# surftemp/cae_tools

Measured on AMD Instinct MI355X. Metric: train images/sec (16x16->256x256, batch 64), higher is better.
Workload: dtype f32

## Files before the change

### cae_tools_amd/csrc/engine.hip

```cpp
#include <hip/hip_runtime.h>

#include <dlfcn.h>

#include <algorithm>
#include <cmath>
#include <cstdio>
#include <cstdlib>
#include <cstring>
#include <map>
#include <string>
#include <tuple>
#include <vector>

#include "cae_hip.h"
#include "kernels_generic.h"
#include "kernels_s2.h"
#include "kernels_last.h"
#include "kernels_rows.h"
#include "kernels_gemm.h"
#include "kernels_igemm.h"
#include "kernels_ctlds.h"
#include "kernels_head.h"
#include "dp_comm.h"
#include "kernels_ctbwd.h"
#include "trunk_api.h"
#include "engine_host.h"

namespace cae {
template __global__ void k_ct_fwd_lds<3, 3>(CtFwd);
template __global__ void k_s2_fwd_rows<8, 4, 1, 2>(S2FwdRows);
template __global__ void k_s2_fwd_rows<4, 2, 2, 1>(S2FwdRows);
template __global__ void k_s2_last_fused<2, 1, 4, 4, 4, true, true>(S2Last);
template __global__ void k_s2_bwd_rows<4, 4, 2, 3, 3, 2, 1, 3>(S2Rows);
template __global__ void k_s2_bwd_rows<8, 2, 4, 3, 3, 4, 2, 1>(S2Rows);
}

using namespace cae;
using namespace cae_internal;

namespace cae_internal {
int ctbwd_launch(const void* args, size_t bytes, unsigned gx, unsigned gy, unsigned gz, size_t lds, hipStream_t s);
}

namespace {
thread_local std::string g_err;
}

void cae_detail_set_error(const char* msg) { g_err = msg; }

namespace {

constexpr float kBnEps = 1e-5f;
constexpr float kBnMomentum = 0.1f;
constexpr int kLossSlots = 1 << 16;

int64_t align_up(int64_t v, int64_t a) { return (v + a - 1) / a * a; }

struct ConvLayer {
    bool transposed;
    int cin, hin, win, cout, hout, wout, kh, kw, stride, opad;
    bool has_bn;
    int bn_index;
    int64_t w_off, b_off, gamma_off, beta_off;
    int64_t rm_off, rv_off;
    int64_t act_off, grad_off;
    int sh_w = -1, sh_b = -1;
    int64_t out_elems() const { return (int64_t)cout * hout * wout; }
    int64_t in_elems() const { return (int64_t)cin * hin * win; }
};

struct FcLayer {
    int nin, nout;
    int64_t w_off, b_off;
    int64_t act_off, grad_off;
    bool relu;
};

}

struct cae_engine {
    std::vector<ConvLayer> enc, dec;
    FcLayer fc[4];
    int fc_size = 0, latent = 0, max_batch = 0;
    int in_c = 0, in_h = 0, in_w = 0, out_c = 0, out_h = 0, out_w = 0;
    TensorTable tab;
    int n_bn = 0;
    std::vector<int64_t> bn_stat_off;
    std::vector<int64_t> bn_saved_off;
    std::vector<int> bn_channels;
    int max_channels = 0;

    int64_t off_state = 0, off_losses = 0, off_zero_begin = 0, off_gradacc = 0, off_zero_end = 0;
    int64_t off_glast = 0, off_sgacc = 0;
    ShardSegs segs{};
    int64_t ws_need = 0;

    float *params = nullptr, *grads = nullptr, *m = nullptr, *v = nullptr, *bufs = nullptr;
    char* ws = nullptr;
    hipStream_t stream = nullptr;
    Hyper hp{1e-3, 0.9, 0.999, 1e-8, 1e-5};
    const float* ds_x[2] = {nullptr, nullptr};
    const float* ds_t[2] = {nullptr, nullptr};
    int64_t ds_n[2] = {0, 0};
    bool graph_mode = true;
    bool lr_stale = true;
    long long captures = 0;
    bool capture_only = false;
    bool use_s2 = true;
    bool variational = false;
    int64_t off_vz = 0, off_vgz = 0, off_zlast = 0;
    cae_internal::TrunkHooks hooks{nullptr, nullptr, nullptr};
    bool gather_fwd = false;
    int ctbwd_mask = 0;
    int ctbwd_auto = 0;
    int64_t off_xbatch = 0;
    bool x_published = false;
    AdamConv0 c0_pending{};
    bool profiling = false;
    struct ProfRec { const char* name; int layer; double bytes; hipEvent_t e0, e1; };
    std::vector<ProfRec> prof;
    std::map<std::tuple<int, int, int, int, const void*, int, int, int, int, int>, hipGraphExec_t> graphs;

    int dp_world = 0, dp_rank = 0;
    RcclApi::comm_t dp_comm = nullptr;
    hipStream_t comm_stream = nullptr;
    hipEvent_t ev_fork = nullptr, ev_join = nullptr;
    bool dp_graph_ok = true;
    bool dp_overlap = true;
    std::vector<int> sync_order;
    size_t sync_pos = 0;
    int64_t bucket_split = 0;

    StepState* state() const { return reinterpret_cast<StepState*>(ws + off_state); }
    double* losses() const { return reinterpret_cast<double*>(ws + off_losses); }
    double* gradacc() const { return reinterpret_cast<double*>(ws + off_gradacc); }
    double* sgacc() const { return reinterpret_cast<double*>(ws + off_sgacc); }
    ShardSegs shard_segs() const {
        ShardSegs r = segs;
        r.base = sgacc();
        return r;
    }
    double* bn_stats(int j) const { return reinterpret_cast<double*>(ws + bn_stat_off[j]); }
    float* bn_saved(int j) const { return reinterpret_cast<float*>(ws + bn_saved_off[j]); }
    float* fptr(int64_t off) const { return reinterpret_cast<float*>(ws + off); }
    void drop_graphs() {
        for (auto& kv : graphs) (void)hipGraphExecDestroy(kv.second);
        graphs.clear();
    }
};

namespace {


BnDesc bn_none() {
    BnDesc d;
    memset(&d, 0, sizeof d);
    d.mode = BN_NONE;
    return d;
}

BnDesc bn_of(const cae_engine* e, const ConvLayer& L, int mode, double count, int update) {
    if (!L.has_bn) return bn_none();
    BnDesc d;
    memset(&d, 0, sizeof d);
    d.mode = mode;
    d.C = L.cout;
    d.stats = e->bn_stats(L.bn_index);
    d.gamma = e->params + L.gamma_off;
    d.beta = e->params + L.beta_off;
    d.rmean = e->bufs + L.rm_off;
    d.rvar = e->bufs + L.rv_off;
    d.saved = e->bn_saved(L.bn_index);
    d.count = count;
    d.inv_count = count > 0.0 ? 1.0 / count : 0.0;
    d.unbias = count > 1.0 ? count / (count - 1.0) : 1.0;
    d.momentum = kBnMomentum;
    d.eps = kBnEps;
    d.update = update;
    return d;
}

Src src_plain(const float* p, int C, int H, int W) {
    Src s;
    memset(&s, 0, sizeof s);
    s.p = p;
    s.C = C;
    s.H = H;
    s.W = W;
    return s;
}

Epi epi_plain(float* out) {
    Epi e;
    memset(&e, 0, sizeof e);
// ... 342 lines not shown
}

constexpr int kLastHB = 4;

struct LastPick { bool vec4, bn; };

int last_strips(const ConvLayer& L) {
    const int qw = (L.wout + 1) / 2;
    const int wmax = L.win > qw - 1 ? L.win : qw - 1;
    return (wmax + kLastStripPx - 1) / kLastStripPx;
}

LastPick choose_last(const ConvLayer& L, bool bn_in) { return LastPick{last_strips(L) == 1 && (L.wout & 3) == 0, bn_in}; }

template <int CIN, int COUT, int KH, int KW>
bool last_fused_launch(S2Last a, LastPick p, hipStream_t s) {
    if constexpr (CIN * COUT * KH * KW <= 72) {
        a.QH = (a.OH + 1) / 2;
        a.QW = (a.OW + 1) / 2;
        const int wmax = a.W > a.QW - 1 ? a.W : a.QW - 1, hmax = a.H > a.QH - 1 ? a.H : a.QH - 1;
        a.strips = (wmax + kLastStripPx - 1) / kLastStripPx;
        a.bands = (hmax + kLastHB - 1) / kLastHB;
        a.total = a.B * a.strips * a.bands;
        const dim3 grid((a.total + 3) / 4);
        if (p.vec4 && p.bn) hipLaunchKernelGGL((k_s2_last_fused<CIN, COUT, KH, KW, kLastHB, true, true>), grid, dim3(256), 0, s, a);
        else if (p.bn) hipLaunchKernelGGL((k_s2_last_fused<CIN, COUT, KH, KW, kLastHB, false, true>), grid, dim3(256), 0, s, a);
        else hipLaunchKernelGGL((k_s2_last_fused<CIN, COUT, KH, KW, kLastHB, false, false>), grid, dim3(256), 0, s, a);
        return true;
    }
    return false;
}

bool last_fused_dispatch(const ConvLayer& L, const S2Last& a, hipStream_t s) {
    const LastPick p = choose_last(L, a.bn_in.mode != BN_NONE);
#define ONE(CI, CO, KH_, KW_) \
    if (L.cin == CI && L.cout == CO && L.kh == KH_ && L.kw == KW_) return last_fused_launch<CI, CO, KH_, KW_>(a, p, s);
#define PAIR(CI, CO) S2_KERNELS(ONE, CI, CO)
    S2_SHAPES(PAIR)
#undef PAIR
#undef ONE
    return false;
}

template <class K>
void head_lds_attr(K kernel, size_t bytes) {
    static size_t granted = 64 * 1024;
    if (bytes > granted) {
        (void)hipFuncSetAttribute(reinterpret_cast<const void*>(kernel), hipFuncAttributeMaxDynamicSharedMemorySize, (int)bytes);
        granted = bytes;
    }
}

template <int KH, int KW>
void ct_fwd_go(const CtFwd& c, dim3 grid, int threads, size_t lds, hipStream_t s) {
    head_lds_attr(k_ct_fwd_lds<KH, KW>, lds);
    hipLaunchKernelGGL((k_ct_fwd_lds<KH, KW>), grid, dim3(threads), lds, s, c);
}

constexpr int kCtFwdMfmas = 24;

bool ct_fwd_plan(const cae_engine* e, int batch, const ConvLayer& L, int layer, CtFwd& c, int& waves, size_t& lds) {
    if (e->gather_fwd || layer >= 31 || L.cin % 4 || L.kh < 3 || L.kw < 3) return false;
    memset(&c, 0, sizeof c);
    c.B = batch; c.Cin = L.cin; c.H = L.hin; c.W = L.win; c.Cout = L.cout; c.OH = L.hout; c.OW = L.wout;
    c.QH = (L.hout + 1) / 2; c.QW = (L.wout + 1) / 2;
    c.PW = c.QW + 1;
    c.plane = ((c.QH + 1) * c.PW) | 1;
    c.tiles = (c.QH * c.QW + 15) / 16;
    const int taps = ((L.kh + 1) / 2 + L.kh / 2) * ((L.kw + 1) / 2 + L.kw / 2);
    const int mf = L.cin * taps / 4;
    int ks = 1;
    while (ks < 8 && mf / ks > kCtFwdMfmas && L.cin % (ks * 2 * 4) == 0) ks *= 2;
    int rt = 8 / ks;
    if (rt > c.tiles) rt = c.tiles;
    if (rt > 4) rt = 4;
    c.ks = ks; c.rt = rt;
    c.tg = (c.tiles + rt - 1) / rt;
    waves = rt * ks;
    lds = ct_fwd_lds_bytes(L.cin, c.plane, L.kh, L.kw, waves, ks);
    return !(lds > 150 * 1024 || c.plane >= kDivSmallMaxD || (long long)L.cin * c.plane >= kDivSmallMaxN);
}

void ct_fwd_launch(cae_engine* e, const StepArgs& a, const ConvLayer& L, int layer, const float* in, const BnDesc& bn_in,
                   float* out, double* stats) {
    CtFwd c;
    int waves = 0;
    size_t lds = 0;
    (void)ct_fwd_plan(e, a.batch, L, layer, c, waves, lds);
    c.in = in; c.bn_in = bn_in; c.w = e->params + L.w_off; c.bias = e->params + L.b_off; c.out = out; c.stats = stats;
    dim3 grid((unsigned)(a.batch * c.tg), (unsigned)((L.cout + 15) / 16));
    ProfScope _p(e, a.train ? "ct_convt_fwd" : "ct_convt_eval", layer, f4((double)a.batch * (L.in_elems() + L.out_elems())));
    if (L.kh == 3 && L.kw == 3) ct_fwd_go<3, 3>(c, grid, 64 * waves, lds, e->stream);
    else if (L.kh == 4 && L.kw == 4) ct_fwd_go<4, 4>(c, grid, 64 * waves, lds, e->stream);
    else if (L.kh == 3 && L.kw == 4) ct_fwd_go<3, 4>(c, grid, 64 * waves, lds, e->stream);
    else ct_fwd_go<4, 3>(c, grid, 64 * waves, lds, e->stream);
}

struct CtBwdPlan { int imgs, groups, wstr; size_t lds; };

bool ct_bwd_plan(const cae_engine* e, int B, const ConvLayer& L, int l, CtBwdPlan& p) {
    if (!(l < 31 && ((e->ctbwd_mask >> l) & 1) && L.kh == 3 && L.kw == 3 && L.stride == 2 && L.cin % 16 == 0 && L.cout % 4 == 0 &&
          L.hout >= 2 * L.hin + 1 && L.wout >= 2 * L.win + 1))
        return false;
    const int HW = L.hin * L.win, OHW = L.hout * L.wout, N = L.cout * 9;
    const int budget = std::min((4 * kCtbG4 * kCtbThreads) / (L.cout * OHW), (4 * kCtbA4 * kCtbThreads) / (16 * HW));
    int imgs = (int)(((int64_t)L.cin * N * B + 149999) / 150000);
    imgs = std::max(1, std::min(std::min(imgs, budget), B));
    p.imgs = imgs;
    p.groups = (B + imgs - 1) / imgs;
    p.wstr = N | 1;
    p.lds = ct_bwd_lds_bytes(L.cin, L.cout, imgs, HW, OHW, p.wstr);
    return budget >= 1 && 16 * N <= 4 * kCtbW4 * kCtbThreads && p.lds <= 152 * 1024 && (int64_t)L.cin * N * p.groups <= 400000;
}


bool head_plan(const cae_engine* e, const StepArgs& a, HeadArgs& h, size_t& lds_bytes) {
    if (!e->use_s2 || a.syncing() || e->variational || (int)e->enc.size() > kHeadMaxEnc) return false;
    memset(&h, 0, sizeof h);
    h.B = a.batch;
    h.n_enc = (int)e->enc.size();
    h.train = a.train ? 1 : 0;
    h.momentum = kBnMomentum;
    h.eps = kBnEps;
    h.st = e->state();
    h.tiles_per_wg = 1;
    double* acc = e->gradacc();
    int64_t top = 0;
    auto take = [&](int64_t floats) {
        top = align_up(top, 4);
        const int64_t o = top;
        top += floats;
        return (int)o;
    };
    h.o_perm = take(a.batch);
    int maxc = 1;
    for (int l = 0; l < h.n_enc; l++) {
        const ConvLayer& L = e->enc[l];
        if (L.cout > kHeadMaxC) return false;
        HeadConv& c = h.enc[l];
        c.cin = L.cin; c.hin = L.hin; c.win = L.win; c.cout = L.cout; c.hout = L.hout; c.wout = L.wout;
        c.kh = L.kh; c.kw = L.kw; c.s = L.stride;
        c.w = e->params + L.w_off; c.bias = e->params + L.b_off;
        c.gamma = e->params + L.gamma_off; c.beta = e->params + L.beta_off;
        c.rmean = e->bufs + L.rm_off; c.rvar = e->bufs + L.rv_off; c.saved = e->bn_saved(L.bn_index);
        c.y = e->fptr(L.act_off);
        {
            const double count = (double)a.batch * L.hout * L.wout;
            c.inv_count = 1.0 / count;
            c.unbias = count > 1.0 ? count / (count - 1.0) : 1.0;
        }
        {
            const int64_t pn = L.beta_off + L.cout - L.w_off, bnn = L.rv_off + L.cout - L.rm_off;
            if (pn > kHeadThreads || bnn > kHeadThreads || pn <= 0 || bnn <= 0 || h.n_seg + 2 > kHeadMaxSeg) return false;
            c.o_w = take(pn);
            c.o_b = c.o_w + (int)(L.b_off - L.w_off);
            c.o_gamma = c.o_w + (int)(L.gamma_off - L.w_off);
            c.o_beta = c.o_w + (int)(L.beta_off - L.w_off);
            c.o_rm = take(bnn);
            c.o_rv = c.o_rm + (int)(L.rv_off - L.rm_off);
            h.seg[h.n_seg++] = HeadSeg{e->params + L.w_off, (int)pn, c.o_w, 0};
            h.seg[h.n_seg++] = HeadSeg{e->bufs + L.rm_off, (int)bnn, c.o_rm, 0};
        }
        c.o_c = take(4 * (int64_t)L.cout);
        if (l + 1 == h.n_enc) c.o_y = take((int64_t)a.batch * L.out_elems());
        if (L.cout > maxc) maxc = L.cout;
    }
    int maxd = 0;
    for (int i = 0; i < 4; i++) {
        const FcLayer& F = e->fc[i];
        HeadFc& f = h.fc[i];
        f.nin = F.nin; f.nout = F.nout; f.relu = F.relu ? 1 : 0;
        f.w = e->params + F.w_off; f.bias = e->params + F.b_off;
// ... 96 lines not shown
    t.ld2 = ld_of(e->fc[2].nout);
    t.ld1 = ld_of(e->fc[1].nout);
    t.ld0 = ld_of(e->fc[0].nout);
    int64_t top = 0;
    auto take = [&](int64_t floats) {
        top = align_up(top, 4);
        const int64_t o = top;
        top += floats;
        return (int)o;
    };
    t.o_c = take(4 * (int64_t)P.cout);
    t.o_red = take(2 * 2 * (int64_t)kHeadWaves);
    t.o_g2 = take(16 * (int64_t)t.ld2 + 32);
    t.o_g1 = take(16 * (int64_t)t.ld1 + 32);
    t.o_g0 = take(16 * (int64_t)t.ld0 + 32);
    t.o_y = take(16 * (int64_t)e->fc[0].nin + 32);
    t.o_gx = take(16 * (int64_t)e->fc[0].nin + 32);
    top = align_up(top, 4);
    t.zero4 = (int)((top - t.o_g2) / 4);
    int64_t wmax = 0;
    for (int i = 0; i < 3; i++) wmax = std::max<int64_t>(wmax, (int64_t)e->fc[i].nout * t.ldw[i]);
    t.o_w = take(wmax + 64);
    t.o_part = take(kHeadWaves * 256);
    lds_bytes = (size_t)align_up(top, 4) * sizeof(float);
    if (lds_bytes > 152 * 1024) return false;
    for (int i = 0; i < 3; i++) t.sp_d[i] = stage_split((e->fc[2 - i].nin + 15) / 16, e->fc[2 - i].nout);
    for (int i = 0; i < 3; i++) t.sp_w[i] = stage_split(((e->fc[2 - i].nout + 15) / 16) * ((e->fc[2 - i].nin + 16) / 16), 16);
    return true;
}

enum DecFwdK {
    DF_FUSED_LAST,
    DF_ROWS,
    DF_S2,
    DF_CT_LDS,
    DF_IG,
    DF_UP
};
enum DecBwdK {
    DB_FUSED_LAST,
    DB_ROWS,
    DB_S2,
    DB_CT_LDS,
    DB_IG,
    DB_GENERIC
};

int s2_fwd_epi(const cae_engine* e, int l, bool train, bool external_loss) {
    if (l + 1 < (int)e->dec.size()) return train ? S2_RAW_STATS : S2_RAW;
    if (external_loss) return S2_RAW;
    return train ? S2_SIGMSE : S2_SIGOUT;
}

bool rows_ok(const cae_engine* e, const ConvLayer& L, int l) {
    return l + 1 < (int)e->dec.size() && l > 0 && e->dec[l - 1].has_bn && rows_bwd_ok(e, L);
}

DecFwdK choose_dec_fwd(const cae_engine* e, const ConvLayer& L, int l, int B, bool train, bool external_loss) {
    const bool last = l + 1 == (int)e->dec.size();
    if (last && train && !external_loss && last_fused_ok(e, L)) return DF_FUSED_LAST;
    if (rows_ok(e, L, l)) return DF_ROWS;
    if (s2_eligible(e, L)) return DF_S2;
    if (e->use_s2 && !last && L.stride == 2 && L.kh <= 4 && L.kw <= 4) {
        CtFwd c;
        int waves = 0;
        size_t lds = 0;
        return ct_fwd_plan(e, B, L, l, c, waves, lds) ? DF_CT_LDS : DF_IG;
    }
    return DF_UP;
}

DecBwdK choose_dec_bwd(const cae_engine* e, const ConvLayer& L, int l, int B, bool external_loss) {
    const bool last = l + 1 == (int)e->dec.size();
    if (last && !external_loss && last_fused_ok(e, L)) return DB_FUSED_LAST;
    if (rows_ok(e, L, l)) return DB_ROWS;
    if (s2_eligible(e, L)) return DB_S2;
    if (e->use_s2) {
        CtBwdPlan p;
        return ct_bwd_plan(e, B, L, l, p) ? DB_CT_LDS : DB_IG;
    }
    return DB_GENERIC;
}

StepTail narrow_tail(cae_engine* e, bool with_step_tail, int batch_inc) {
    StepTail t = step_tail_of(e, batch_inc, 1);
    if (!with_step_tail) {
        t.zero_extra = nullptr;
        t.zero_extra_n = 0;
        t.st = nullptr;
    }
    return t;
}

int dp_allreduce_grads(cae_engine* e, int64_t lo, int64_t hi, hipStream_t on) {
    if (hi <= lo) return CAE_OK;
    NCCL_TRY(rccl().AllReduce(e->grads + lo, e->grads + lo, (size_t)(hi - lo), RcclApi::kFloat32, RcclApi::kSum, e->dp_comm, on));
    return CAE_OK;
}

bool dp_overlap(const cae_engine* e, const StepArgs& a) { return e->dp_overlap && !a.dp_sync; }

bool dp_single_collective(const cae_engine* e, const StepArgs& a) { return !dp_overlap(e, a) && !a.dp_sync; }

int dp_first_bucket(cae_engine* e, const StepArgs& a) {
    if (!a.dp || dp_single_collective(e, a)) return CAE_OK;
    const int64_t lo = e->bucket_split, hi = e->tab.n_param;
    const bool overlap = dp_overlap(e, a);
    hipStream_t on = overlap ? e->comm_stream : e->stream;
    if (overlap) {
        HIP_TRY(hipEventRecord(e->ev_fork, e->stream));
        HIP_TRY(hipStreamWaitEvent(e->comm_stream, e->ev_fork, 0));
    }
    {
        ProfScope _p(e, "dp_narrow_bucket0", 0, 12.0 * (hi - lo), on);
        hipLaunchKernelGGL(k_narrow_range, dim3(grid1(hi - lo)), dim3(256), 0, on, (long long)lo, (long long)hi, e->grads,
                           e->shard_segs(), narrow_tail(e, false, 0));
    }
    if (int rc = dp_allreduce_grads(e, lo, hi, on)) return rc;
    if (overlap) HIP_TRY(hipEventRecord(e->ev_join, e->comm_stream));
    return CAE_OK;
}

int dp_finish_step(cae_engine* e, const StepArgs& a) {
    hipStream_t s = e->stream;
    const int64_t lo = 0, hi = dp_single_collective(e, a) ? e->tab.n_param : e->bucket_split;
    {
        ProfScope _p(e, "dp_narrow_bucket1", 0, 12.0 * (hi - lo));
        hipLaunchKernelGGL(k_narrow_range, dim3(grid1(hi - lo > 0 ? hi - lo : 1)), dim3(256), 0, s, (long long)lo, (long long)hi,
                           e->grads, e->shard_segs(), narrow_tail(e, true, a.inc()));
    }
    if (dp_overlap(e, a)) HIP_TRY(hipStreamWaitEvent(s, e->ev_join, 0));
    if (int rc = dp_allreduce_grads(e, lo, hi, s)) return rc;
    StepTail none;
    memset(&none, 0, sizeof none);
    ProfScope _p(e, "adam", 0, 28.0 * e->tab.n_param);
    hipLaunchKernelGGL(k_adam, dim3(grid1(e->tab.n_param)), dim3(256), 0, s, (long long)e->tab.n_param, e->params,
                       (const float*)e->grads, e->m, e->v, e->hp, (const StepState*)e->state(), e->shard_segs(), none, 0,
                       std::log(e->hp.beta1), std::log(e->hp.beta2), AdamConv0{});
    return CAE_OK;
}

int launch_forward(cae_engine* e, const StepArgs& a) {
    hipStream_t s = e->stream;
    const int B = a.batch;
    const StepState* st = e->state();
    const int act_mode = a.train ? BN_BATCH : BN_RUNNING;

    HeadArgs head;
    size_t head_lds = 0;
    const bool fused_head = a.part == 0 && head_plan(e, a, head, head_lds);
    if (fused_head) {
        head.x = a.x_direct ? a.x_direct : e->ds_x[a.which];
        head.perm = a.x_direct ? nullptr : a.perm;
        head.use_cursor = a.x_direct ? 0 : 1;
        head.bump_adam = a.train ? 1 : 0;
        const int T = (e->fc[3].nout + 15) / 16;
        double bytes = 0;
        for (auto& L : e->enc) bytes += f4((double)B * (L.in_elems() + L.out_elems()));
        for (int i = 0; i < 4; i++) bytes += f4((double)B * (e->fc[i].nin + e->fc[i].nout) + (double)e->fc[i].nin * e->fc[i].nout);
        head_lds_attr(k_head_fwd, head_lds);
        e->x_published = false;
        if (a.train) {
            head.clear0 = e->bn_stats(e->enc[0].bn_index);
            head.clear0_n = kStatShards * e->enc[0].cout * 4;
            if (a.adam_follows) {
                head.xbatch = e->fptr(e->off_xbatch);
// ... 42 lines not shown
        const int fc_lo = a.part == 2 ? 2 : 0, fc_hi = a.part == 1 ? 2 : 4;
        for (int i = fc_lo; i < fc_hi; i++) {
            const FcLayer& F = e->fc[i];
            ProfScope _p(e, e->use_s2 ? "linear_fwd_mfma" : "linear_fwd", i, f4((double)B * (F.nin + F.nout) + (double)F.nin * F.nout));
            if (e->use_s2) {
                GemmArgs ga;
                memset(&ga, 0, sizeof ga);
                ga.M = B; ga.N = F.nout; ga.K = F.nin;
                ga.A = in; ga.sa_m = F.nin; ga.sa_k = 1;
                ga.B = e->params + F.w_off; ga.sb_k = 1; ga.sb_n = F.nin;
                ga.C = e->fptr(F.act_off); ga.sc_m = F.nout; ga.sc_n = 1;
                ga.epi = GE_STORE;
                ga.bias = e->params + F.b_off;
                ga.relu = F.relu ? 1 : 0;
                ga.bn_a = i == 0 ? bni : bn_none();
                ga.hw_a = hw;
                ga.bn_c = bn_none();
                const int tiles = ((B + 15) / 16) * ((F.nout + 15) / 16);
                hipLaunchKernelGGL(k_gemm16, dim3(tiles), dim3(256), gemm_lds(i == 0 ? P.cout : 0), s, ga);
            } else {
                hipLaunchKernelGGL(k_lin_fwd, dim3(grid1((int64_t)B * F.nout)), dim3(256), lds_bytes(i == 0 ? P.cout : 0, 0),
                                   s, B, F.nin, F.nout, in, i == 0 ? bni : bn_none(), hw, e->params + F.w_off,
                                   e->params + F.b_off, F.relu ? 1 : 0, e->fptr(F.act_off));
            }
            in = e->fptr(F.act_off);
            if (i == 1 && e->variational) {
                if (!e->hooks.reparam) return fail(CAE_ERR_STATE, "trunk engine without a reparameterisation hook");
                e->hooks.reparam(e->hooks.user, s, in, B, e->latent, a.train ? 1 : 0, e->fptr(e->off_vz));
                in = e->fptr(e->off_vz);
            }
        }
        if (a.part == 1) {
            HIP_TRY(hipMemcpyAsync(a.z_out, e->fptr(e->fc[1].act_off), sizeof(float) * (size_t)B * e->fc[1].nout, hipMemcpyDeviceToDevice, s));
            return CAE_OK;
        }
    }
    for (size_t l = 0; l < e->dec.size(); l++) {
        const ConvLayer& L = e->dec[l];
        const bool last = l + 1 == e->dec.size();
        ConvGeom g{B, L.cin, L.hin, L.win, L.cout, L.hout, L.wout, L.kh, L.kw, L.stride};
        Src small;
        BnDesc bns = bn_none();
        if (l == 0) {
            small = src_plain(e->fptr(e->fc[3].act_off), L.cin, L.hin, L.win);
        } else {
            const ConvLayer& P = e->dec[l - 1];
            small = src_plain(e->fptr(P.act_off), L.cin, L.hin, L.win);
            bns = bn_of(e, P, act_mode, (double)a.bn_batch * P.hout * P.wout, 1);
        }
        Epi ep;
        if (!last) {
            ep = epi_plain(e->fptr(L.act_off));
            if (a.train) {
                ep.kind = EPI_STATS;
                ep.stats = e->bn_stats(L.bn_index);
                ep.stats_C = L.cout;
            }
        } else {
            memset(&ep, 0, sizeof ep);
            ep.inv_count = (float)(1.0 / ((double)a.global_batch * L.cout * L.hout * L.wout));
            ep.losses = e->losses();
            ep.perm = a.perm;
            ep.use_cursor = a.use_cursor ? 1 : 0;
            if (a.train) {
                ep.kind = EPI_SIGMSE;
                ep.out = e->fptr(e->off_glast);
                ep.target = e->ds_t[a.which];
                ep.bias_acc = e->gradacc() + L.b_off;
            } else {
                ep.kind = EPI_SIGOUT;
                ep.yhat = a.yhat;
                ep.target = a.want_loss ? e->ds_t[a.which] : nullptr;
            }
        }
        if (last && a.external_loss) {
            ep = epi_plain(e->fptr(e->off_zlast));
        }
        const DecFwdK fk = choose_dec_fwd(e, L, (int)l, B, a.train, a.external_loss);
        if (fk == DF_FUSED_LAST) continue;
        if (fk == DF_ROWS) {
            S2FwdRows f;
            memset(&f, 0, sizeof f);
            f.B = B; f.H = L.hin; f.W = L.win; f.OH = L.hout; f.OW = L.wout;
            f.in = small.p; f.bn_in = bns;
            f.w = e->params + L.w_off; f.bias = e->params + L.b_off;
            f.out = ep.out;
            f.stats = a.train ? ep.stats : nullptr;
            ProfScope _p(e, a.train ? "s2_convt_fwd" : "s2_convt_eval", (int)l, f4((double)B * (L.in_elems() + L.out_elems())));
            rows_fwd_launch(L, f, s);
            if (a.train)
                if (int rc = sync_bn_table(e, a, L.bn_index)) return rc;
            continue;
        }
        if (fk == DF_S2) {
            S2Fwd f;
            memset(&f, 0, sizeof f);
            f.B = B; f.H = L.hin; f.W = L.win; f.OH = L.hout; f.OW = L.wout;
            f.in = small.p;
            f.w = e->params + L.w_off;
            f.bias = e->params + L.b_off;
            f.bn_in = bns;
            f.st = st;
            if (!last) {
                f.out = ep.out;
                f.stats = ep.stats;
                f.epi = a.train ? S2_RAW_STATS : S2_RAW;
            } else if (a.external_loss) {
                f.out = ep.out;
                f.epi = S2_RAW;
            } else {
                f.out = a.train ? ep.out : ep.yhat;
                f.target = ep.target;
                f.perm = ep.perm;
                f.use_cursor = ep.use_cursor;
                f.losses = ep.losses;
                f.inv_count = ep.inv_count;
                f.bias_acc = e->sgacc() + L.sh_b;
                f.bias_stride = e->segs.n;
                f.epi = a.train ? S2_SIGMSE : S2_SIGOUT;
            }
            ProfScope _p(e, last ? (a.train ? "s2_convt_last_fwd_loss" : "s2_convt_last_eval") : (a.train ? "s2_convt_fwd" : "s2_convt_eval"), (int)l,
                         f4((double)B * (L.in_elems() + L.out_elems() * (last && (a.train || a.want_loss) ? 2.0 : 1.0))));
            if (!s2_fwd_dispatch(L, f, s))
                return fail(CAE_ERR_STATE, "decoder layer %d: no k_s2_fwd kernel for the chosen variant", (int)l);
            if (a.train && !last)
                if (int rc = sync_bn_table(e, a, L.bn_index)) return rc;
            continue;
        }
        if (fk == DF_CT_LDS) {
            ct_fwd_launch(e, a, L, (int)l, small.p, bns, ep.out, a.train ? ep.stats : nullptr);
            if (a.train)
                if (int rc = sync_bn_table(e, a, L.bn_index)) return rc;
            continue;
        }
        if (fk == DF_IG) {
            IgFwd f;
            memset(&f, 0, sizeof f);
            f.B = B; f.Cin = L.cin; f.H = L.hin; f.W = L.win; f.Cout = L.cout; f.OH = L.hout; f.OW = L.wout;
            f.KH = L.kh; f.KW = L.kw; f.QH = (L.hout + 1) / 2; f.QW = (L.wout + 1) / 2;
            f.in = small.p; f.bn_in = bns; f.w = e->params + L.w_off; f.bias = e->params + L.b_off;
            f.out = ep.out; f.stats = a.train ? ep.stats : nullptr;
            const int mtiles = (B * f.QH * f.QW + 15) / 16;
            f.ksplit = L.cin >= 48 ? 4 : (L.cin >= 24 ? 2 : 1);
            {
                const int waves_m = 4 / f.ksplit, target = 1024;
                int tpw = (mtiles * 4 + waves_m * target - 1) / (waves_m * target);
                f.tiles_per_wave = tpw < 1 ? 1 : (tpw > 8 ? 8 : tpw);
            }
            const int per_block = (4 / f.ksplit) * f.tiles_per_wave;
            dim3 grid((mtiles + per_block - 1) / per_block, 4, (L.cout + 15) / 16);
            ProfScope _p(e, a.train ? "ig_convt_fwd" : "ig_convt_eval", (int)l, f4((double)B * (L.in_elems() + L.out_elems())));
            hipLaunchKernelGGL(k_ig_fwd_s2, grid, dim3(256), (64 + 1024) * sizeof(float) + (size_t)(L.cin + 1) * sizeof(float4), s, f);
            if (a.train)
                if (int rc = sync_bn_table(e, a, L.bn_index)) return rc;
            continue;
        }
        dim3 grid(grid1((int64_t)B * L.hout * L.wout), L.cout);
        ProfScope _p(e, last ? (a.train ? "dec_convt_last_fwd_loss" : "dec_convt_last_eval") : (a.train ? "dec_convt_fwd" : "dec_convt_eval"), (int)l,
                     f4((double)B * (L.in_elems() + L.out_elems() * (last && (a.train || a.want_loss) ? 2.0 : 1.0))));
        hipLaunchKernelGGL(k_up, grid, dim3(256), lds_bytes(L.cin, L.cout), s, g, small, bns, e->params + L.w_off,
                           e->params + L.b_off, ep, bn_none(), st);
        if (a.train && !last)
            if (int rc = sync_bn_table(e, a, L.bn_index)) return rc;
    }
    return CAE_OK;
}

int launch_backward(cae_engine* e, const StepArgs& a) {
    hipStream_t s = e->stream;
    const int B = a.batch;
    const StepState* st = e->state();
    double* acc = e->gradacc();

    for (int l = (int)e->dec.size() - 1; l >= 0; l--) {
        const ConvLayer& L = e->dec[l];
        const bool last = l + 1 == (int)e->dec.size();
        const DecBwdK bk = choose_dec_bwd(e, L, l, B, a.external_loss);
        ConvGeom g{B, L.cin, L.hin, L.win, L.cout, L.hout, L.wout, L.kh, L.kw, L.stride};
        Src gy;
        BnDesc bng = bn_none();
        if (last) {
            gy = src_plain(e->fptr(e->off_glast), L.cout, L.hout, L.wout);
        } else {
            gy = src_plain(e->fptr(L.grad_off), L.cout, L.hout, L.wout);
            gy.q = e->fptr(L.act_off);
            bng = bn_of(e, L, BN_BWD, (double)a.bn_batch * L.hout * L.wout, 0);
        }
        Src ain;
        BnDesc bna = bn_none();
        if (l == 0) {
            ain = src_plain(e->fptr(e->fc[3].act_off), L.cin, L.hin, L.win);
        } else {
            const ConvLayer& P = e->dec[l - 1];
            ain = src_plain(e->fptr(P.act_off), L.cin, L.hin, L.win);
            bna = bn_of(e, P, BN_SAVED, 0, 0);
        }
        if (bk == DB_FUSED_LAST) {
            S2Last f;
            memset(&f, 0, sizeof f);
            f.B = B; f.H = L.hin; f.W = L.win; f.OH = L.hout; f.OW = L.wout;
            f.in = ain.p;
            f.w = e->params + L.w_off;
            f.bias = e->params + L.b_off;
            f.target = e->ds_t[a.which];
            f.perm = a.perm;
            f.use_cursor = a.use_cursor ? 1 : 0;
            f.st = st;
            f.losses = e->losses();
            f.inv_count = (float)(1.0 / ((double)a.global_batch * L.cout * L.hout * L.wout));
            f.bias_acc = e->sgacc() + L.sh_b;
            f.wacc = e->sgacc() + L.sh_w;
            f.acc_stride = e->segs.n;
            if (l == 0) {
                f.bn_in = bn_none();
                f.gin = e->fptr(e->fc[3].grad_off);
            } else {
                const ConvLayer& P = e->dec[l - 1];
                f.bn_in = bn_of(e, P, BN_BATCH, (double)a.bn_batch * P.hout * P.wout, 1);
                f.gin = e->fptr(P.grad_off);
                f.stats_in = e->bn_stats(P.bn_index);
            }
            ProfScope _p(e, "s2_convt_last_fused", l, f4((double)B * (L.in_elems() * 2.0 + L.out_elems())));
            if (!last_fused_dispatch(L, f, s))
                return fail(CAE_ERR_STATE, "decoder layer %d: no k_s2_last_fused kernel for the chosen variant", (int)l);
            if (l > 0)
                if (int rc = sync_bn_table(e, a, e->dec[l - 1].bn_index)) return rc;
            continue;
        }
        if (bk == DB_ROWS) {
            const ConvLayer& P = e->dec[l - 1];
            S2Rows f;
            memset(&f, 0, sizeof f);
            f.B = B; f.H = L.hin; f.W = L.win; f.OH = L.hout; f.OW = L.wout;
            f.g = gy.p; f.yout = gy.q; f.bn_out = bng;
            f.ain = ain.p; f.bn_in = bna;
            f.w = e->params + L.w_off;
            f.gin = e->fptr(P.grad_off);
            f.stats_in = e->bn_stats(P.bn_index);
            f.wacc = e->sgacc() + L.sh_w;
            f.wacc_stride = e->segs.n;
            f.bg.stats = e->bn_stats(L.bn_index);
            f.bg.gamma_acc = acc + L.gamma_off;
            f.bg.beta_acc = acc + L.beta_off;
            f.bg.C = L.cout;
            f.bg.scale = 1.0 / a.world;
            ProfScope _p(e, "s2_convt_bwd", l, f4((double)B * (L.out_elems() * 2.0 + L.in_elems() * 2.0)));
            rows_bwd_launch(L, f, s);
            if (int rc = sync_bn_table(e, a, P.bn_index)) return rc;
            continue;
        }
        if (bk == DB_S2) {
            S2Bwd f;
            memset(&f, 0, sizeof f);
            f.B = B; f.H = L.hin; f.W = L.win; f.OH = L.hout; f.OW = L.wout;
            f.g = gy.p;
            f.yout = gy.q;
            f.bn_out = bng;
            f.ain = ain.p;
            f.bn_in = bna;
            f.w = e->params + L.w_off;
            f.wacc = e->sgacc() + L.sh_w;
            f.wacc_stride = e->segs.n;
            if (l == 0) {
                f.gin = e->fptr(e->fc[3].grad_off);
            } else {
                const ConvLayer& P = e->dec[l - 1];
                f.gin = e->fptr(P.grad_off);
                f.stats_in = e->bn_stats(P.bn_index);
            }
            if (L.has_bn) {
                f.bg.stats = e->bn_stats(L.bn_index);
                f.bg.gamma_acc = acc + L.gamma_off;
                f.bg.beta_acc = acc + L.beta_off;
                f.bg.C = L.cout;
                f.bg.scale = 1.0 / a.world;
            }
            ProfScope _p(e, "s2_convt_bwd", l,
                         f4((double)B * (L.out_elems() * (last ? 1.0 : 2.0) + L.in_elems() * 2.0)));
            if (!s2_bwd_dispatch(L, f, s))
                return fail(CAE_ERR_STATE, "decoder layer %d: no k_s2_bwd kernel for the chosen variant", (int)l);
            if (l > 0)
                if (int rc = sync_bn_table(e, a, e->dec[l - 1].bn_index)) return rc;
            continue;
        }
        if (bk == DB_CT_LDS) {
            CtBwdPlan cp;
            (void)ct_bwd_plan(e, B, L, l, cp);
            const int HW = L.hin * L.win, OHW = L.hout * L.wout;
            const int imgs = cp.imgs, groups = cp.groups, wstr = cp.wstr;
            const size_t lds = cp.lds;
            CtBwd c;
            memset(&c, 0, sizeof c);
            c.B = B; c.Cin = L.cin; c.H = L.hin; c.W = L.win; c.Cout = L.cout; c.OH = L.hout; c.OW = L.wout;
            c.imgs = imgs; c.wstr = wstr;
            c.g = gy.p; c.yout = gy.q; c.bn_out = bng;
            c.ain = ain.p; c.bn_in = bna;
            c.w = e->params + L.w_off;
            if (L.sh_w >= 0) {
                c.wacc = e->sgacc() + L.sh_w;
                c.wacc_stride = e->segs.n;
            } else {
                c.wacc = acc + L.w_off;
            }
            if (l == 0) {
                c.gin = e->fptr(e->fc[3].grad_off);
            } else {
                const ConvLayer& P = e->dec[l - 1];
                c.gin = e->fptr(P.grad_off);
                c.stats_prev = e->bn_stats(P.bn_index);
            }
            if (L.has_bn) {
                c.bg.stats = e->bn_stats(L.bn_index);
                c.bg.gamma_acc = acc + L.gamma_off;
                c.bg.beta_acc = acc + L.beta_off;
                c.bg.C = L.cout;
                c.bg.scale = 1.0 / a.world;
            }
            ProfScope _p(e, "ct_convt_bwd", l,
                         f4((double)B * (L.out_elems() * (last ? 1.0 : 2.0) + L.in_elems() * (l == 0 ? 1.0 : 2.0))));
            int parts = std::max(1, std::min(8, 256 / (groups * (L.cin / 16))));
            size_t lds_launch = lds;
            if (imgs == 1 && parts > 1) {
                const int hb = (L.hin + parts - 1) / parts, bands = (L.hin + hb - 1) / hb;
                const int gstr = (2 * hb + 1) * L.wout, astr = hb * L.win;
                if (bands > 1 && L.cout * gstr <= 8 * kCtbThreads && 16 * astr <= 2 * kCtbThreads) {
                    c.bands = bands;
                    c.hb = hb;
                    parts = bands;
                    lds_launch = (32 * (size_t)kCtbWaves + 4 * (size_t)(L.cin + L.cout) + (size_t)L.cout * gstr + 4 + 16 * (size_t)astr + 4 +
                                  16 * (size_t)wstr + 3 * (size_t)astr + (size_t)kCtbWaves * 16 * 17 + 8) * sizeof(float);
                }
            }
            if (cae_internal::ctbwd_launch(&c, sizeof c, (unsigned)groups, (unsigned)(L.cin / 16), (unsigned)parts, lds_launch, s))
                return fail(CAE_ERR_ARG, "k_ct_bwd_lds: argument layout mismatch");
            if (l > 0)
                if (int rc = sync_bn_table(e, a, e->dec[l - 1].bn_index)) return rc;
            continue;
        }
        if (bk == DB_IG) {
            IgWgrad fw;
            memset(&fw, 0, sizeof fw);
            fw.B = B; fw.Cin = L.cin; fw.H = L.hin; fw.W = L.win; fw.Cout = L.cout; fw.OH = L.hout; fw.OW = L.wout;
            fw.KH = L.kh; fw.KW = L.kw; fw.S = L.stride;
            fw.ain = ain.p; fw.bn_in = bna; fw.g = gy.p; fw.yout = gy.q; fw.bn_out = bng;
            fw.wacc = acc + L.w_off;
            if (L.has_bn) {
                fw.bg.stats = e->bn_stats(L.bn_index);
                fw.bg.gamma_acc = acc + L.gamma_off;
                fw.bg.beta_acc = acc + L.beta_off;
                fw.bg.C = L.cout;
                fw.bg.scale = 1.0 / a.world;
            }
            const int wtiles = ((L.cin + 15) / 16) * ((L.cout * L.kh * L.kw + 15) / 16);
            const int steps = (B * L.hin * L.win + 3) / 4;
            int chunks = 2048 / wtiles;
            if (chunks < 1) chunks = 1;
            int per = (steps + chunks - 1) / chunks;
            per = (per + 31) / 32 * 32;
            chunks = (steps + per - 1) / per;
            fw.ksteps_per_block = per;

            IgDgrad fd;
            memset(&fd, 0, sizeof fd);
            fd.B = B; fd.Cin = L.cin; fd.H = L.hin; fd.W = L.win; fd.Cout = L.cout; fd.OH = L.hout; fd.OW = L.wout;
            fd.KH = L.kh; fd.KW = L.kw; fd.S = L.stride;
            fd.g = gy.p; fd.yout = gy.q; fd.bn_out = bng; fd.w = e->params + L.w_off;
            if (l == 0) {
                fd.gin = e->fptr(e->fc[3].grad_off);
            } else {
                const ConvLayer& P = e->dec[l - 1];
                fd.gin = e->fptr(P.grad_off);
                fd.yprev = e->fptr(P.act_off);
                fd.bn_prev = bn_of(e, P, BN_SAVED, 0, 0);
                fd.stats_prev = e->bn_stats(P.bn_index);
            }
            const int mtiles = (B * L.hin * L.win + 15) / 16;
            const int ksteps = (L.cout * L.kh * L.kw + 3) / 4;
            fd.ksplit = ksteps > 24 ? 4 : (ksteps > 12 ? 2 : 1);
            fd.tiles_per_wave = mtiles >= 8192 ? 2 : 1;
            const int per_block = (4 / fd.ksplit) * fd.tiles_per_wave;
            const int d_gx = (mtiles + per_block - 1) / per_block, d_gy = (L.cin + 15) / 16;
            const size_t lds_d = (128 + 1024) * sizeof(float) + (size_t)(L.cin + L.cout + 1) * sizeof(float4) +
                                 (size_t)L.cout * L.kh * L.kw * 2 * sizeof(int);
            const size_t lds_w = 1024 * sizeof(float) + (size_t)(L.cin + L.cout + 1) * sizeof(float4);
            ProfScope _p(e, "ig_convt_bwd_pair", l,
                         f4((double)B * (L.out_elems() * (last ? 1.0 : 2.0) + L.in_elems() * (l == 0 ? 1.0 : 2.0))));
            int d_group = (per * 4) / (per_block * 16);
            if (d_group < 1) d_group = 1;
            const int w_n8 = (chunks + 7) / 8, d_n8 = ((d_gx + d_group - 1) / d_group + 7) / 8;
            hipLaunchKernelGGL(k_ig_bwd_pair, dim3(8 * wtiles * w_n8 + 8 * d_n8 * d_group * d_gy), dim3(256),
                               lds_d > lds_w ? lds_d : lds_w, s, fw, fd, wtiles, chunks, w_n8, d_gx, d_gy, d_group);
            if (l > 0)
                if (int rc = sync_bn_table(e, a, e->dec[l - 1].bn_index)) return rc;
            continue;
        }
        {
            const int64_t nw = (int64_t)L.cin * L.cout * L.kh * L.kw;
            const int64_t pos = (int64_t)B * L.hin * L.win;
            const int ppb = wgrad_ppb(pos, nw);
            BnGradOut bg;
            memset(&bg, 0, sizeof bg);
            if (L.has_bn) {
                bg.stats = e->bn_stats(L.bn_index);
                bg.gamma_acc = acc + L.gamma_off;
                bg.beta_acc = acc + L.beta_off;
                bg.C = L.cout;
                bg.scale = 1.0 / a.world;
            }
            dim3 grid((unsigned)nw, (unsigned)((pos + ppb - 1) / ppb));
            ProfScope _p(e, "dec_convt_wgrad", l, f4((double)B * (L.in_elems() + L.out_elems() * (last ? 1.0 : 2.0))));
            hipLaunchKernelGGL(k_wgrad, grid, dim3(256), lds_bytes(L.cin, L.cout), s, g, ain, bna, gy, bng,
                               acc + L.w_off, ppb, bg, st);
        }
        {
// ... 222 lines not shown

int launch_one(cae_engine* e, int op, const StepArgs& a);

int launch_op(cae_engine* e, int op, const StepArgs& a) {
    for (int i = 0; i < a.nsteps; i++)
        if (int rc = launch_one(e, op, a)) return rc;
    return CAE_OK;
}

int launch_one(cae_engine* e, int op, const StepArgs& a) {
    hipStream_t s = e->stream;
    {
        ProfScope _cal(e, "event_pair", -1, 0.0);
    }
    if (op == OP_DP_TRAIN) {
        e->sync_pos = 0;
        if (a.batch > 0) {
            int rc = launch_forward(e, a);
            if (rc) return rc;
            rc = launch_backward(e, a);
            if (rc) return rc;
        } else {
            hipLaunchKernelGGL(k_bump_adam, dim3(1), dim3(1), 0, s, e->state());
            if (a.dp_sync)
                for (int bn : e->sync_order)
                    if (int rc = sync_bn_table(e, a, bn)) return rc;
            if (int rc = dp_first_bucket(e, a)) return rc;
        }
        if (a.dp_sync && e->sync_pos != e->sync_order.size())
            return fail(CAE_ERR_STATE, "SyncBN: %zu of %zu tables all-reduced", e->sync_pos, e->sync_order.size());
        if (int rc = dp_finish_step(e, a)) return rc;
    } else if (op == OP_TRAIN || op == OP_FWDBWD) {
        StepArgs af = a;
        af.adam_follows = op == OP_TRAIN;
        memset(&e->c0_pending, 0, sizeof e->c0_pending);
        int rc = launch_forward(e, af);
        if (rc) return rc;
        rc = launch_backward(e, af);
        if (rc) return rc;
        if (op == OP_TRAIN) {
            ProfScope _p(e, "adam", 0, 32.0 * e->tab.n_param);
            AdamConv0 c0 = e->c0_pending;
            StepTail tl = step_tail_of(e, a.inc(), 1);
            int nreg = grid1(e->tab.n_param), grid = nreg;
            if (c0.on) {
                const long long skip = (long long)kStatShards * c0.C * 4;
                tl.zero_extra += skip;
                tl.zero_extra_n -= skip;
                c0.n_regular = nreg;
                grid = nreg + c0.nw;
            }
            hipLaunchKernelGGL(k_adam, dim3(grid), dim3(256), 0, s, (long long)e->tab.n_param, e->params,
                               (const float*)nullptr, e->m, e->v, e->hp, (const StepState*)e->state(), e->shard_segs(),
                               tl, 0, std::log(e->hp.beta1), std::log(e->hp.beta2), c0);
        } else {
            hipLaunchKernelGGL(k_acc_to_f32, dim3(grid1(e->tab.n_param)), dim3(256), 0, s, (long long)e->tab.n_param, e->grads,
                               e->shard_segs(), step_tail_of(e, a.inc(), 1));
        }
    } else if (op == OP_EVAL) {
        int rc = launch_forward(e, a);
        if (rc) return rc;
        if (a.use_cursor) hipLaunchKernelGGL(k_advance, dim3(1), dim3(1), 0, s, e->state(), a.inc(), 1, 0);
    } else if (op == OP_ADAM) {
        StepTail none;
        memset(&none, 0, sizeof none);
        hipLaunchKernelGGL(k_adam, dim3(grid1(e->tab.n_param)), dim3(256), 0, s, (long long)e->tab.n_param, e->params,
                           (const float*)e->grads, e->m, e->v, e->hp, (const StepState*)e->state(), e->shard_segs(),
                           none, 0, std::log(e->hp.beta1), std::log(e->hp.beta2), AdamConv0{});
    }
    HIP_TRY(hipGetLastError());
    return CAE_OK;
}

int push_lr(cae_engine* e) {
    if (!e->lr_stale || !e->ws) return CAE_OK;
    hipLaunchKernelGGL(k_set_lr, dim3(1), dim3(1), 0, e->stream, e->state(), e->hp.lr);
    HIP_TRY(hipGetLastError());
    e->lr_stale = false;
    return CAE_OK;
}

int run_op(cae_engine* e, int op, const StepArgs& a, bool cacheable) {
    if (int rc = push_lr(e)) return rc;
    if (!e->graph_mode || !cacheable || e->stream == nullptr || e->profiling)
        return e->capture_only ? CAE_OK : launch_op(e, op, a);
    auto key = std::make_tuple(op, a.which, a.batch, a.global_batch, (const void*)a.perm, a.nsteps, a.cursor_inc,
                               a.dp_sync ? 1 : 0, a.bn_batch, a.world);
    auto it = e->graphs.find(key);
    if (it == e->graphs.end()) {
        hipGraph_t graph = nullptr;
        HIP_TRY(hipStreamBeginCapture(e->stream, hipStreamCaptureModeThreadLocal));
        int rc = launch_op(e, op, a);
        hipError_t ce = hipStreamEndCapture(e->stream, &graph);
        if (rc) {
            if (graph) (void)hipGraphDestroy(graph);
            return rc;
        }
        if (ce != hipSuccess) return fail(CAE_ERR_HIP, "hipStreamEndCapture: %s", hipGetErrorString(ce));
        hipGraphExec_t exec = nullptr;
        hipError_t ie = hipGraphInstantiate(&exec, graph, nullptr, nullptr, 0);
        (void)hipGraphDestroy(graph);
        if (ie != hipSuccess) return fail(CAE_ERR_HIP, "hipGraphInstantiate: %s", hipGetErrorString(ie));
        it = e->graphs.emplace(key, exec).first;
        e->captures += 1;
    }
    if (e->capture_only) return CAE_OK;
    HIP_TRY(hipGraphLaunch(it->second, e->stream));
    return CAE_OK;
}

int check_ready(const cae_engine* e, int which, int batch, bool need_target) {
    if (!e) return fail(CAE_ERR_ARG, "null engine");
    if (!e->ws) return fail(CAE_ERR_STATE, "cae_bind has not been called");
    if (batch < 1 || batch > e->max_batch) return fail(CAE_ERR_ARG, "batch %d outside [1, %d]", batch, e->max_batch);
    if (which < 0 || which > 1) return fail(CAE_ERR_ARG, "dataset index %d is not 0 or 1", which);
    if (!e->ds_x[which]) return fail(CAE_ERR_STATE, "dataset %d has not been set", which);
    if (need_target && !e->ds_t[which]) return fail(CAE_ERR_STATE, "dataset %d has no target array", which);
    return CAE_OK;
}

}


extern "C" {

const char* cae_last_error(void) { return g_err.c_str(); }
int cae_abi_version(void) { return 1; }

static int engine_create_impl(const cae_layer_spec* enc, int n_enc, const cae_layer_spec* dec, int n_dec, int fc_size,
                              int latent_size, int max_batch, bool variational, cae_engine** out);

int cae_engine_create(const cae_layer_spec* enc, int n_enc, const cae_layer_spec* dec, int n_dec, int fc_size,
                      int latent_size, int max_batch, cae_engine** out) {
    return engine_create_impl(enc, n_enc, dec, n_dec, fc_size, latent_size, max_batch, false, out);
}

static int engine_create_impl(const cae_layer_spec* enc, int n_enc, const cae_layer_spec* dec, int n_dec, int fc_size,
                              int latent_size, int max_batch, bool variational, cae_engine** out) {
    if (!enc || !dec || !out || n_enc < 1 || n_dec < 1) return fail(CAE_ERR_ARG, "need >=1 encoder and decoder layer");
    if (fc_size < 1 || latent_size < 1 || max_batch < 1) return fail(CAE_ERR_ARG, "fc/latent/max_batch must be >= 1");
    cae_engine* e = new cae_engine();
    e->fc_size = fc_size;
    e->latent = latent_size;
    e->max_batch = max_batch;
    e->variational = variational;
    auto bad = [&](const char* msg, int i) {
        delete e;
        return fail(CAE_ERR_ARG, "layer %d: %s", i, msg);
    };
    for (int i = 0; i < n_enc; i++) {
        const cae_layer_spec& s = enc[i];
        if (s.stride < 1 || s.k_h < 1 || s.k_w < 1 || s.in_c < 1 || s.out_c < 1) return bad("bad encoder spec", i);
        if (s.in_h < s.k_h || s.in_w < s.k_w) return bad("encoder kernel larger than input", i);
        if (s.out_h != (s.in_h - s.k_h) / s.stride + 1 || s.out_w != (s.in_w - s.k_w) / s.stride + 1)
            return bad("encoder output size != floor((in-k)/stride)+1", i);
        if (i > 0 && (enc[i - 1].out_c != s.in_c || enc[i - 1].out_h != s.in_h || enc[i - 1].out_w != s.in_w))
            return bad("encoder layer input does not match previous output", i);
    }
    for (int i = 0; i < n_dec; i++) {
        const cae_layer_spec& s = dec[i];
        if (s.stride < 1 || s.k_h < 1 || s.k_w < 1 || s.in_c < 1 || s.out_c < 1) return bad("bad decoder spec", i);
        if (s.output_padding < 0 || (s.output_padding >= s.stride && s.output_padding > 0))
            return bad("output_padding must be smaller than stride", i);
        if (s.out_h != (s.in_h - 1) * s.stride + s.k_h + s.output_padding ||
            s.out_w != (s.in_w - 1) * s.stride + s.k_w + s.output_padding)
            return bad("decoder output size != (in-1)*stride+k+output_padding", i);
// ... 57 lines not shown
        L.transposed = true;
        L.cin = s.in_c; L.hin = s.in_h; L.win = s.in_w;
        L.cout = s.out_c; L.hout = s.out_h; L.wout = s.out_w;
        L.kh = s.k_h; L.kw = s.k_w; L.stride = s.stride; L.opad = s.output_padding;
        L.has_bn = i != n_dec - 1;
        L.bn_index = L.has_bn ? bn++ : -1;
        const std::string c = "dec/decoder_conv." + std::to_string(3 * i);
        const std::string b = "dec/decoder_conv." + std::to_string(3 * i + 1);
        L.w_off = e->tab.add(c + ".weight", 0, {L.cin, L.cout, L.kh, L.kw});
        L.b_off = e->tab.add(c + ".bias", 0, {L.cout});
        if (L.has_bn) {
            L.gamma_off = e->tab.add(b + ".weight", 0, {L.cout});
            L.beta_off = e->tab.add(b + ".bias", 0, {L.cout});
            L.rm_off = e->tab.add(b + ".running_mean", 1, {L.cout});
            L.rv_off = e->tab.add(b + ".running_var", 1, {L.cout});
        }
        e->dec.push_back(L);
    }
    e->tab.close();
    e->n_bn = bn;
    e->bucket_split = e->fc[3].w_off;
    for (auto& L : e->enc) e->sync_order.push_back(L.bn_index);
    for (auto& L : e->dec)
        if (L.has_bn) e->sync_order.push_back(L.bn_index);
    for (int l = n_dec - 1; l >= 1; l--) e->sync_order.push_back(e->dec[l - 1].bn_index);
    e->sync_order.push_back(e->enc.back().bn_index);
    for (int l = n_enc - 1; l >= 1; l--) e->sync_order.push_back(e->enc[l - 1].bn_index);

    {
        int n = 0;
        for (size_t l = 0; l < e->dec.size(); l++) {
            ConvLayer& L = e->dec[l];
            const bool ctb = l < 31 && L.transposed && L.stride == 2 && L.kh == 3 && L.kw == 3 && L.cin % 16 == 0 && L.cout % 4 == 0 &&
                             L.cin == 16 && L.cin * L.cout * 9 <= 2048;
            if (l == 0) e->ctbwd_auto = 0;
            if (ctb) e->ctbwd_auto |= 1 << l;
            e->ctbwd_mask = e->ctbwd_auto;
            if ((!s2_shape_ok(L) && !ctb) || e->segs.nseg + 2 > 12) continue;
            const int nw = L.cin * L.cout * L.kh * L.kw;
            L.sh_w = n;
            e->segs.seg[e->segs.nseg++] = ShardSeg{L.w_off, nw, n};
            n += (nw + 3) / 4 * 4;
            if (l + 1 == e->dec.size()) {
                L.sh_b = n;
                e->segs.seg[e->segs.nseg++] = ShardSeg{L.b_off, L.cout, n};
                n += (L.cout + 3) / 4 * 4;
            }
        }
        e->segs.n = n;
    }

    Carver carve{256};
    e->off_state = carve(sizeof(StepState));
    e->off_losses = carve((int64_t)kLossSlots * kStatShards * sizeof(double));
    carve(1024 * 3 * sizeof(double));
    e->bn_stat_off.resize(bn);
    e->bn_saved_off.resize(bn);
    e->bn_channels.resize(bn);
    e->off_zero_begin = carve.top;
    auto reg_bn = [&](const ConvLayer& L) {
        if (!L.has_bn) return;
        e->bn_channels[L.bn_index] = L.cout;
        e->bn_stat_off[L.bn_index] = carve((int64_t)kStatShards * L.cout * 4 * sizeof(double));
        if (L.cout > e->max_channels) e->max_channels = L.cout;
    };
    for (auto& L : e->enc) reg_bn(L);
    for (auto& L : e->dec) reg_bn(L);
    e->off_gradacc = carve(e->tab.n_param * (int64_t)sizeof(double));
    e->off_sgacc = carve((int64_t)kStatShards * (e->segs.n > 0 ? e->segs.n : 4) * (int64_t)sizeof(double));
    e->off_zero_end = carve.top;
    for (auto& L : e->enc) e->bn_saved_off[L.bn_index] = carve((int64_t)L.cout * 2 * sizeof(float));
    for (auto& L : e->dec)
        if (L.has_bn) e->bn_saved_off[L.bn_index] = carve((int64_t)L.cout * 2 * sizeof(float));
    const int64_t mb = max_batch;
    for (auto& L : e->enc) {
        L.act_off = carve(mb * L.out_elems() * 4);
        L.grad_off = carve(mb * L.out_elems() * 4);
    }
    for (int i = 0; i < 4; i++) {
        e->fc[i].act_off = carve(mb * e->fc[i].nout * 4);
        e->fc[i].grad_off = carve(mb * e->fc[i].nout * 4);
    }
    for (auto& L : e->dec) {
        if (!L.has_bn) continue;
        L.act_off = carve(mb * L.out_elems() * 4);
        L.grad_off = carve(mb * L.out_elems() * 4);
    }
    e->off_glast = carve(mb * e->dec.back().out_elems() * 4);
    e->off_xbatch = carve((mb * e->enc[0].in_elems() + e->enc[0].cout) * 4);
    if (variational) {
        e->off_vz = carve(mb * latent_size * 4);
        e->off_vgz = carve(mb * latent_size * 4);
        e->off_zlast = carve(mb * e->dec.back().out_elems() * 4);
    }
    e->ws_need = carve.top;
    for (auto& L : e->enc)
        if (L.cin > e->max_channels) e->max_channels = L.cin;
    for (auto& L : e->dec)
        if (L.cin > e->max_channels) e->max_channels = L.cin;
    if (lds_bytes(e->max_channels, e->max_channels) > 60 * 1024) {
        delete e;
        return fail(CAE_ERR_ARG, "channel count %d exceeds the LDS constant table", e->max_channels);
    }
    *out = e;
    return CAE_OK;
}

void cae_engine_destroy(cae_engine* e) {
    if (!e) return;
    e->drop_graphs();
    (void)cae_dp_shutdown(e);
    delete e;
}

int64_t cae_param_count(const cae_engine* e) { return e ? e->tab.n_param : 0; }
int64_t cae_buffer_count(const cae_engine* e) { return e ? e->tab.n_buf : 0; }
int cae_tensor_count(const cae_engine* e) { return e ? e->tab.count() : 0; }
int cae_tensor_info(const cae_engine* e, int index, cae_tensor_info_t* out) {
    return e ? e->tab.info(index, out) : fail(CAE_ERR_ARG, "tensor index out of range");
}
int64_t cae_workspace_bytes(const cae_engine* e) { return e ? e->ws_need : 0; }
int cae_loss_slots(const cae_engine*) { return kLossSlots; }

int cae_bind(cae_engine* e, float* params, float* grads, float* exp_avg, float* exp_avg_sq, float* buffers,
             void* workspace, int64_t workspace_bytes) {
    if (!e || !params || !grads || !exp_avg || !exp_avg_sq || !buffers || !workspace)
        return fail(CAE_ERR_ARG, "cae_bind: null pointer");
    if (workspace_bytes < e->ws_need)
        return fail(CAE_ERR_ARG, "workspace too small: %lld < %lld", (long long)workspace_bytes, (long long)e->ws_need);
    if (((uintptr_t)workspace & 255) != 0) return fail(CAE_ERR_ARG, "workspace must be 256-byte aligned");
    e->drop_graphs();
    e->lr_stale = true;
    e->params = params;
    e->grads = grads;
    e->m = exp_avg;
    e->v = exp_avg_sq;
    e->bufs = buffers;
    e->ws = static_cast<char*>(workspace);
    return CAE_OK;
}

int cae_set_stream(cae_engine* e, void* hip_stream) {
    if (!e) return fail(CAE_ERR_ARG, "null engine");
    if (e->stream != (hipStream_t)hip_stream) {
        e->drop_graphs();
        e->lr_stale = true;
    }
    e->stream = (hipStream_t)hip_stream;
    return CAE_OK;
}

int cae_set_graph_mode(cae_engine* e, int enabled) {
    if (!e) return fail(CAE_ERR_ARG, "null engine");
    e->graph_mode = enabled != 0;
    if (!e->graph_mode) e->drop_graphs();
    return CAE_OK;
}

int cae_set_capture_only(cae_engine* e, int enabled) {
    if (!e) return fail(CAE_ERR_ARG, "null engine");
    e->capture_only = enabled != 0;
    return CAE_OK;
}

int cae_set_kernel_mode(cae_engine* e, int specialised) {
    if (!e) return fail(CAE_ERR_ARG, "null engine");
    const int ctb = (specialised & 2) ? 0x7fffffff : e->ctbwd_auto;
    const bool gather = (specialised & 4) != 0;
    if (e->use_s2 != ((specialised & 1) != 0) || ctb != e->ctbwd_mask || gather != e->gather_fwd) e->drop_graphs();
    e->use_s2 = (specialised & 1) != 0;
    e->ctbwd_mask = ctb;
    e->gather_fwd = gather;
    return CAE_OK;
}

int cae_set_hyper(cae_engine* e, double lr, double beta1, double beta2, double eps, double weight_decay) {
    if (!e) return fail(CAE_ERR_ARG, "null engine");
    Hyper h{lr, beta1, beta2, eps, weight_decay};
    if (h.beta1 != e->hp.beta1 || h.beta2 != e->hp.beta2 || h.eps != e->hp.eps || h.wd != e->hp.wd) e->drop_graphs();
    e->hp = h;
    e->lr_stale = true;
    return push_lr(e);
}

int cae_set_lr(cae_engine* e, double lr) {
    if (!e) return fail(CAE_ERR_ARG, "null engine");
    e->hp.lr = lr;
    e->lr_stale = true;
    return push_lr(e);
}

int cae_set_dataset(cae_engine* e, int which, const float* x, const float* t, int64_t n) {
    if (!e || which < 0 || which > 1 || !x || n < 1) return fail(CAE_ERR_ARG, "cae_set_dataset: bad argument");
    if (e->ds_x[which] != x || e->ds_t[which] != t) e->drop_graphs();
    e->ds_x[which] = x;
    e->ds_t[which] = t;
    e->ds_n[which] = n;
    return CAE_OK;
}

int cae_set_cursor(cae_engine* e, int64_t batch_start, int loss_slot) {
    if (!e || !e->ws) return fail(CAE_ERR_STATE, "cae_bind has not been called");
    if (loss_slot < 0 || loss_slot >= kLossSlots) return fail(CAE_ERR_ARG, "loss slot out of range");
    hipLaunchKernelGGL(k_set_state, dim3(1), dim3(1), 0, e->stream, e->state(), (long long)batch_start, loss_slot, 1, 0, 0);
    HIP_TRY(hipGetLastError());
    return CAE_OK;
}

int cae_set_adam_step(cae_engine* e, int completed_steps) {
    if (!e || !e->ws) return fail(CAE_ERR_STATE, "cae_bind has not been called");
    hipLaunchKernelGGL(k_set_state, dim3(1), dim3(1), 0, e->stream, e->state(), 0LL, 0, 0, completed_steps, 1);
    HIP_TRY(hipGetLastError());
    return CAE_OK;
}

int cae_train_step(cae_engine* e, int which, const int32_t* perm, int batch) {
    int rc = check_ready(e, which, batch, true);
    if (rc) return rc;
    StepArgs a{which, perm, batch, batch, batch, true, true, nullptr, nullptr, true};
    return run_op(e, OP_TRAIN, a, true);
}

int cae_train_steps(cae_engine* e, int which, const int32_t* perm, int batch, int nsteps) {
    int rc = check_ready(e, which, batch, true);
    if (rc) return rc;
    if (nsteps < 1 || nsteps > 4096) return fail(CAE_ERR_ARG, "nsteps %d outside [1, 4096]", nsteps);
    StepArgs a{which, perm, batch, batch, batch, true, true, nullptr, nullptr, true};
    a.nsteps = nsteps;
    return run_op(e, OP_TRAIN, a, true);
}

int cae_eval_steps(cae_engine* e, int which, const int32_t* perm, int batch, int nsteps) {
    int rc = check_ready(e, which, batch, true);
    if (rc) return rc;
    if (nsteps < 1 || nsteps > 4096) return fail(CAE_ERR_ARG, "nsteps %d outside [1, 4096]", nsteps);
    StepArgs a{which, perm, batch, batch, batch, false, true, nullptr, nullptr, true};
    a.nsteps = nsteps;
    return run_op(e, OP_EVAL, a, true);
}

int cae_forward_backward(cae_engine* e, int which, const int32_t* perm, int batch, int global_batch) {
    int rc = check_ready(e, which, batch, true);
    if (rc) return rc;
    if (global_batch < batch) return fail(CAE_ERR_ARG, "global_batch < batch");
    StepArgs a{which, perm, batch, global_batch, batch, true, true, nullptr, nullptr, true};
    return run_op(e, OP_FWDBWD, a, true);
}

int cae_forward_backward_sync(cae_engine* e, int which, const int32_t* perm, int batch, int global_batch, int world,
                              cae_allreduce_fn fn, void* user) {
    int rc = check_ready(e, which, batch, true);
    if (rc) return rc;
// ... 239 lines not shown
    a.z_in = z;
    return run_op(e, OP_EVAL, a, false);
}

int cae_read_losses(cae_engine* e, int first, int count, double* host_out) {
    if (!e || !e->ws) return fail(CAE_ERR_STATE, "cae_bind has not been called");
    if (first < 0 || count < 0 || first + count > kLossSlots || !host_out) return fail(CAE_ERR_ARG, "bad loss range");
    if (count == 0) return CAE_OK;
    std::vector<double> raw((size_t)count * kStatShards);
    double* dev = e->losses() + (size_t)first * kStatShards;
    HIP_TRY(hipMemcpyAsync(raw.data(), dev, raw.size() * sizeof(double), hipMemcpyDeviceToHost, e->stream));
    HIP_TRY(hipMemsetAsync(dev, 0, raw.size() * sizeof(double), e->stream));
    HIP_TRY(hipStreamSynchronize(e->stream));
    for (int i = 0; i < count; i++) {
        double t = 0.0;
        for (int sh = 0; sh < kStatShards; sh++) t += raw[(size_t)i * kStatShards + sh];
        host_out[i] = t;
    }
    return CAE_OK;
}

int cae_sync(cae_engine* e) {
    if (!e) return fail(CAE_ERR_ARG, "null engine");
    HIP_TRY(hipStreamSynchronize(e->stream));
    return CAE_OK;
}

int cae_graph_count(const cae_engine* e) { return e ? (int)e->graphs.size() : 0; }
int64_t cae_graph_captures(const cae_engine* e) { return e ? (int64_t)e->captures : 0; }

namespace {
struct RoctxApi {
    int (*push)(const char*) = nullptr;
    int (*pop)() = nullptr;
    bool tried = false;
    void load() {
        if (tried) return;
        tried = true;
        for (const char* name : {"librocprofiler-sdk-roctx.so", "librocprofiler-sdk-roctx.so.1", "libroctx64.so", "libroctx64.so.4"}) {
            if (void* h = dlopen(name, RTLD_NOW | RTLD_GLOBAL)) {
                push = reinterpret_cast<int (*)(const char*)>(dlsym(h, "roctxRangePushA"));
                pop = reinterpret_cast<int (*)()>(dlsym(h, "roctxRangePop"));
                if (push && pop) return;
                push = nullptr;
                pop = nullptr;
            }
        }
    }
};
RoctxApi g_roctx;
}

int cae_trace_range_push(const char* name) {
    g_roctx.load();
    if (!g_roctx.push || !name) return 0;
    g_roctx.push(name);
    return 1;
}

int cae_trace_range_pop(void) {
    if (!g_roctx.pop) return 0;
    g_roctx.pop();
    return 1;
}

int64_t cae_debug_read(cae_engine* e, const char* what, int index, void* host_out, int64_t cap) {
    if (!e || !e->ws || !what || !host_out) return fail(CAE_ERR_ARG, "cae_debug_read: bad argument");
    const void* src = nullptr;
    int64_t n = 0, esz = 4;
    const int64_t mb = e->max_batch;
    const std::string w(what);
    const int n_enc = (int)e->enc.size(), n_dec = (int)e->dec.size();
    auto conv_at = [&](int i) -> const ConvLayer* {
        if (i < 0) return nullptr;
        if (i < n_enc) return &e->enc[i];
        if (i < n_enc + n_dec - 1) return &e->dec[i - n_enc];
        return nullptr;
    };
    if (w == "act" || w == "grad") {
        const ConvLayer* L = conv_at(index);
        if (!L) return fail(CAE_ERR_ARG, "layer index out of range");
        src = e->ws + (w == "act" ? L->act_off : L->grad_off);
        n = mb * L->out_elems();
    } else if (w == "glast") {
        src = e->ws + e->off_glast;
        n = mb * e->dec.back().out_elems();
    } else if (w == "latent") {
        src = e->ws + e->fc[1].act_off;
        n = mb * e->fc[1].nout;
    } else if (w == "fc") {
        if (index < 0 || index > 3) return fail(CAE_ERR_ARG, "fc index out of range");
        src = e->ws + e->fc[index].act_off;
        n = mb * e->fc[index].nout;
    } else if (w == "fcgrad") {
        if (index < 0 || index > 3) return fail(CAE_ERR_ARG, "fc index out of range");
        src = e->ws + e->fc[index].grad_off;
        n = mb * e->fc[index].nout;
    } else if (w == "grad_acc") {
        src = e->gradacc();
        n = e->tab.n_param;
        esz = 8;
    } else if (w == "bn_stats") {
        if (index < 0 || index >= e->n_bn) return fail(CAE_ERR_ARG, "bn index out of range");
        src = e->bn_stats(index);
        n = (int64_t)kStatShards * e->bn_channels[index] * 4;
        esz = 8;
    } else {
        return fail(CAE_ERR_ARG, "unknown tensor '%s'", what);
    }
    if (n > cap) n = cap;
    HIP_TRY(hipStreamSynchronize(e->stream));
    HIP_TRY(hipMemcpy(host_out, src, (size_t)(n * esz), hipMemcpyDeviceToHost));
    return n;
}

int cae_debug_launch_floor(cae_engine* e, int n, double* micros_per_kernel) {
    if (!e || !e->ws || !e->stream || n < 1 || !micros_per_kernel) return fail(CAE_ERR_ARG, "cae_debug_launch_floor: bad argument");
    hipGraph_t graph = nullptr;
    hipGraphExec_t exec = nullptr;
    HIP_TRY(hipStreamBeginCapture(e->stream, hipStreamCaptureModeThreadLocal));
    for (int i = 0; i < n; i++) hipLaunchKernelGGL(k_advance, dim3(1), dim3(1), 0, e->stream, e->state(), 0, 0, 0);
    HIP_TRY(hipStreamEndCapture(e->stream, &graph));
    HIP_TRY(hipGraphInstantiate(&exec, graph, nullptr, nullptr, 0));
    hipEvent_t e0, e1;
    HIP_TRY(hipEventCreate(&e0));
    HIP_TRY(hipEventCreate(&e1));
    for (int i = 0; i < 3; i++) HIP_TRY(hipGraphLaunch(exec, e->stream));
    HIP_TRY(hipEventRecord(e0, e->stream));
    const int reps = 10;
    for (int i = 0; i < reps; i++) HIP_TRY(hipGraphLaunch(exec, e->stream));
    HIP_TRY(hipEventRecord(e1, e->stream));
    HIP_TRY(hipStreamSynchronize(e->stream));
    float ms = 0;
    HIP_TRY(hipEventElapsedTime(&ms, e0, e1));
    *micros_per_kernel = (double)ms * 1000.0 / (reps * (double)n);
    (void)hipEventDestroy(e0);
    (void)hipEventDestroy(e1);
    (void)hipGraphExecDestroy(exec);
    (void)hipGraphDestroy(graph);
    return CAE_OK;
}

int cae_profile_begin(cae_engine* e) {
    if (!e || !e->ws) return fail(CAE_ERR_STATE, "cae_bind has not been called");
    for (auto& r : e->prof) {
        (void)hipEventDestroy(r.e0);
        (void)hipEventDestroy(r.e1);
    }
    e->prof.clear();
    e->profiling = true;
    return CAE_OK;
}

int cae_profile_end(cae_engine* e, cae_profile_rec* out, int capacity) {
    if (!e) return fail(CAE_ERR_ARG, "null engine");
    e->profiling = false;
    HIP_TRY(hipStreamSynchronize(e->stream));
    int n = 0;
    for (auto& r : e->prof) {
        float ms = 0.f;
        hipError_t rc = hipEventElapsedTime(&ms, r.e0, r.e1);
        if (rc == hipSuccess && out && n < capacity) {
            memset(&out[n], 0, sizeof out[n]);
            snprintf(out[n].name, sizeof out[n].name, "%s", r.name);
            out[n].layer = r.layer;
            out[n].micros = (double)ms * 1000.0;
            out[n].bytes = r.bytes;
            n++;
        }
        (void)hipEventDestroy(r.e0);
        (void)hipEventDestroy(r.e1);
    }
    e->prof.clear();
    return n;
}

int cae_debug_plan(const cae_engine* e, int batch, int train, char* out, int64_t out_bytes) {
    if (!e || !out || out_bytes < 1) return fail(CAE_ERR_ARG, "cae_debug_plan: bad argument");
    if (batch < 1 || batch > e->max_batch) return fail(CAE_ERR_ARG, "cae_debug_plan: batch %d outside 1 .. %d", batch, e->max_batch);
    const bool tr = train != 0, ext = e->variational;
    const StepArgs a{0, nullptr, batch, batch, batch, tr, true, nullptr, nullptr, false};
    std::string s;
    char line[256];
    {
        HeadArgs h;
        size_t lds = 0;
        snprintf(line, sizeof line, "head fwd=%s\n", head_plan(e, a, h, lds) ? "fused" : "layers");
        s += line;
    }
    static const char* const kEpiName[] = {"raw_stats", "sigmse", "sigout", "raw"};
    for (int l = 0; l < (int)e->dec.size(); l++) {
        const ConvLayer& L = e->dec[l];
        const int ci = L.cin, co = L.cout, kh = L.kh, kw = L.kw;
        char f[128], b[128];
        switch (choose_dec_fwd(e, L, l, batch, tr, ext)) {
            case DF_FUSED_LAST: {
                const LastPick p = choose_last(L, l > 0 && e->dec[l - 1].has_bn);
                snprintf(f, sizeof f, "last_fused<%d,%d,%d,%d> hb=%d vec4=%d bn=%d", ci, co, kh, kw, kLastHB, (int)p.vec4, (int)p.bn);
                break;
            }
            case DF_ROWS: {
                const RowsPick p = choose_rows_fwd(L);
                snprintf(f, sizeof f, "s2_fwd_rows<%d,%d,%d,%d>", ci, co, p.hb, 64 / p.lw);
                break;
            }
            case DF_S2: {
                const int epi = s2_fwd_epi(e, l, tr, ext);
                const S2FwdPick p = choose_s2_fwd(L, batch, epi);
                const char* fam = p.k == S2F_CS ? "s2_fwd_cs" : (p.k == S2F_QUAD ? "s2_fwd" : "s2_fwd2");
                snprintf(f, sizeof f, "%s<%d,%d,%d,%d,%d> epi=%s", fam, ci, co, kh, kw, p.tw, kEpiName[epi]);
                break;
            }
            case DF_CT_LDS: snprintf(f, sizeof f, "ct_fwd_lds<%d,%d>", kh, kw); break;
            case DF_IG: snprintf(f, sizeof f, "ig_fwd_s2"); break;
            case DF_UP: snprintf(f, sizeof f, "up"); break;
        }
        if (!tr) {
            snprintf(b, sizeof b, "-");
        } else {
            switch (choose_dec_bwd(e, L, l, batch, ext)) {
                case DB_FUSED_LAST: snprintf(b, sizeof b, "(fused)"); break;
                case DB_ROWS: {
                    const RowsPick p = choose_rows_bwd(L);
                    snprintf(b, sizeof b, "s2_bwd_rows<%d,%d,%d,3,3,%d,%d,%d>", ci, ci == 4 ? 4 : 2, co, p.hb, 64 / p.lw, p.d);
                    break;
                }
                case DB_S2: {
                    const S2BwdPick p = choose_s2_bwd(L);
                    if (p.k == S2B_DIRECT) snprintf(b, sizeof b, "s2_bwd2<%d,%d,%d,%d,%d>", ci, co, kh, kw, p.tw);
                    else if (p.k == S2B_SPLIT) snprintf(b, sizeof b, "s2_bwd_split<%d,%d,%d,%d,%d,%d>", ci, p.ct, co, kh, kw, p.tw);
                    else snprintf(b, sizeof b, "s2_bwd<%d,%d,%d,%d,%d>", ci, p.ct, co, kh, kw);
                    break;
                }
                case DB_CT_LDS: snprintf(b, sizeof b, "ct_bwd_lds"); break;
                case DB_IG: snprintf(b, sizeof b, "ig_bwd_pair"); break;
                case DB_GENERIC: snprintf(b, sizeof b, "wgrad+down"); break;
            }
        }
        snprintf(line, sizeof line, "dec%d fwd=%s bwd=%s\n", l, f, b);
        s += line;
    }
    {
        TailArgs t;
        size_t lds = 0;
        snprintf(line, sizeof line, "tail bwd=%s\n", !tr ? "-" : (tail_plan(e, a, t, lds) ? "fused" : "layers"));
        s += line;
    }
    if ((int64_t)s.size() + 1 > out_bytes)
        return fail(CAE_ERR_ARG, "cae_debug_plan: the report needs %zu bytes, got %lld", s.size() + 1, (long long)out_bytes);
    memcpy(out, s.c_str(), s.size() + 1);
    return CAE_OK;
}


int cae_scan_f32(const float* x, int64_t n, void* hip_stream, double* out3) {
    if (!x || n < 1 || !out3) return fail(CAE_ERR_ARG, "cae_scan_f32: bad argument");
    hipStream_t s = (hipStream_t)hip_stream;
    int blocks = (int)((n + 256 * 16 - 1) / (256 * 16));
    if (blocks > 1024) blocks = 1024;
    if (blocks < 1) blocks = 1;
    double* part = nullptr;
    HIP_TRY(hipMalloc(&part, (size_t)blocks * 3 * sizeof(double)));
    hipLaunchKernelGGL(k_scan, dim3(blocks), dim3(256), 0, s, x, (long long)n, part);
    std::vector<double> host((size_t)blocks * 3);
    hipError_t ce = hipMemcpyAsync(host.data(), part, host.size() * sizeof(double), hipMemcpyDeviceToHost, s);
    if (ce == hipSuccess) ce = hipStreamSynchronize(s);
    (void)hipFree(part);
    if (ce != hipSuccess) return fail(CAE_ERR_HIP, "cae_scan_f32: %s", hipGetErrorString(ce));
    double cnt = 0, lo = INFINITY, hi = -INFINITY;
    for (int i = 0; i < blocks; i++) {
        cnt += host[3 * i];
        lo = std::fmin(lo, host[3 * i + 1]);
        hi = std::fmax(hi, host[3 * i + 2]);
    }
    out3[0] = cnt;
    out3[1] = lo;
    out3[2] = hi;
    return CAE_OK;
}

int cae_normalise_pack_rows(const float* src, int64_t n, int c_src, int64_t hw, float* dst, int c_dst, int c_off,
                            float vmin, float range, int enable, const int32_t* dst_row_dev, void* hip_stream) {
    if (!src || !dst || n < 1 || c_src < 1 || hw < 1 || c_off < 0 || c_off + c_src > c_dst)
        return fail(CAE_ERR_ARG, "cae_normalise_pack: bad argument");
    if (n > 0x7fffffffLL) return fail(CAE_ERR_ARG, "cae_normalise_pack: more than 2^31 - 1 rows");
    const long long total = (long long)n * c_src * hw;
    int blocks = (int)((total + 256 * 8 - 1) / (256 * 8));
    if (blocks > 8192) blocks = 8192;
    hipLaunchKernelGGL(k_normalise_pack, dim3(blocks), dim3(256), 0, (hipStream_t)hip_stream, src, total, c_src,
                       (long long)hw, dst, c_dst, c_off, vmin, range, enable, (const int*)dst_row_dev);
    HIP_TRY(hipGetLastError());
    return CAE_OK;
}

int cae_normalise_pack(const float* src, int64_t n, int c_src, int64_t hw, float* dst, int c_dst, int c_off,
                       float vmin, float range, int enable, void* hip_stream) {
    return cae_normalise_pack_rows(src, n, c_src, hw, dst, c_dst, c_off, vmin, range, enable, nullptr, hip_stream);
}

int cae_invert_permutation(const int32_t* perm_dev, int64_t n, int32_t* inverse_dev, void* hip_stream) {
    if (!perm_dev || !inverse_dev || n < 1 || n > 0x7fffffffLL) return fail(CAE_ERR_ARG, "cae_invert_permutation: bad argument");
    hipLaunchKernelGGL(k_invert_perm, dim3((unsigned)((n + 255) / 256)), dim3(256), 0, (hipStream_t)hip_stream,
                       (const int*)perm_dev, (long long)n, (int*)inverse_dev);
    HIP_TRY(hipGetLastError());
    return CAE_OK;
}

int cae_denormalise_f64(const float* y, int64_t n, double vmin, double range, double* out, void* hip_stream) {
    if (!y || !out || n < 1) return fail(CAE_ERR_ARG, "cae_denormalise_f64: bad argument");
    int blocks = (int)((n + 256 * 8 - 1) / (256 * 8));
    if (blocks > 8192) blocks = 8192;
    hipLaunchKernelGGL(k_denorm_f64, dim3(blocks), dim3(256), 0, (hipStream_t)hip_stream, y, (long long)n, vmin, range, out);
    HIP_TRY(hipGetLastError());
    return CAE_OK;
}

int cae_metric_sums(const float* y, const float* actual, const float* mask, int64_t n_inst, int64_t inst_elems,
                    double vmin, double range, double* sums, void* hip_stream) {
    if (!y || !actual || !sums || n_inst < 1 || inst_elems < 1 || n_inst > 65535)
        return fail(CAE_ERR_ARG, "cae_metric_sums: bad argument");
    hipStream_t s = (hipStream_t)hip_stream;
    HIP_TRY(hipMemsetAsync(sums, 0, (size_t)n_inst * 8 * sizeof(double), s));
    int chunks = (int)((inst_elems + 256 * 16 - 1) / (256 * 16));
    if (chunks > 64) chunks = 64;
    hipLaunchKernelGGL(k_metric_sums, dim3(chunks, (unsigned)n_inst), dim3(256), 0, s, y, actual, mask,
                       (long long)inst_elems, vmin, range, sums);
    HIP_TRY(hipGetLastError());
    return CAE_OK;
}
// ... 207 lines not shown
```

### cae_tools_amd/csrc/kernels_ctbwd.h

```cpp
#pragma once
#include "kernels_gemm.h"

namespace cae {

struct CtBwd {
    int B, Cin, H, W, Cout, OH, OW;
    int imgs;
    int bands, hb;
    int wstr;
    const float* g;
    const float* yout;
    BnDesc bn_out;
    const float* ain;
    BnDesc bn_in;
    const float* w;
    float* gin;
    double* stats_prev;
    double* wacc;
    long long wacc_stride;
    BnGradOut bg;
};

constexpr int kCtbThreads = 512;
constexpr int kCtbWaves = kCtbThreads / 64;
constexpr int kCtbG4 = 7;
constexpr int kCtbA4 = 2;
constexpr int kCtbW4 = 3;
constexpr int kCtbKChunk = 64;

inline size_t ct_bwd_lds_bytes(int Cin, int Cout, int imgs, int HW, int OHW, int wstr) {
    size_t floats = 32 * (size_t)kCtbWaves;
    floats += 4 * (size_t)(Cin + Cout);
    floats += (size_t)imgs * Cout * OHW;
    floats += (size_t)imgs * 16 * HW;
    floats += 16 * (size_t)wstr;
    floats += 3 * (size_t)imgs * HW;
    floats += (size_t)kCtbWaves * 16 * 17;
    return (floats + 8) * sizeof(float);
}

#ifdef CAE_CTBWD_KERNEL
template <bool BAND>
__device__ __forceinline__ void ct_bwd_body(const CtBwd& a) {
    extern __shared__ double lds_d[];
    float* lstat = reinterpret_cast<float*>(lds_d);
    float4* cout4 = reinterpret_cast<float4*>(lstat + 32 * kCtbWaves);
    float4* cin4 = cout4 + a.Cout;
    const int HW = a.H * a.W, OHW = a.OH * a.OW, KK = 9, N = a.Cout * KK;
    const int tid = threadIdx.x, wv = tid >> 6, lane = tid & 63;
    const int r = lane & 15, q = lane >> 4;
    const int b0 = blockIdx.x * a.imgs, cb = blockIdx.y;
    const int nimg = BAND ? 1 : min(a.imgs, a.B - b0);
    const int y0 = BAND ? (int)blockIdx.z * a.hb : 0;
    const int nrow = BAND ? min(a.hb, a.H - y0) : a.H;
    const int P = nimg * nrow * a.W;
    const int grows = BAND ? 2 * nrow + 1 : a.OH;
    const int gstr = grows * a.OW;
    const int astr = nrow * a.W;
    float* gimg = reinterpret_cast<float*>(cin4 + a.Cin);
    float* araw = gimg + ((nimg * a.Cout * gstr + 3) & ~3);
    float* wl = araw + ((nimg * 16 * astr + 3) & ~3);
    int* pos_g = reinterpret_cast<int*>(wl + 16 * a.wstr);
    int* pos_a = pos_g + P;
    int* pos_o = pos_a + P;
    float* tiles = reinterpret_cast<float*>(pos_o + P);
    const bool designated = blockIdx.x == 0 && blockIdx.y == 0 && blockIdx.z == 0;
    const bool bwd = a.bn_out.mode == BN_BWD, act = a.bn_in.mode != BN_NONE;
    const float inv_hw = 1.0f / (float)(nrow * a.W), inv_w = 1.0f / (float)a.W, inv_gstr = 1.0f / (float)gstr,
                inv_cout = 1.0f / (float)a.Cout, inv_astr = 1.0f / (float)astr;

    constexpr int NG = BAND ? 8 : kCtbG4, NA = BAND ? 2 : kCtbA4;
    using GT = typename std::conditional<BAND, float, f32x4>::type;
    const int n_g = BAND ? a.Cout * gstr : nimg * a.Cout * OHW / 4;
    GT gv[NG], yv[NG];
    if constexpr (BAND) {
        const float* gb = a.g + ((size_t)b0 * a.Cout * a.OH + 2 * y0) * a.OW;
        const float* yb = bwd ? a.yout + ((size_t)b0 * a.Cout * a.OH + 2 * y0) * a.OW : gb;
#pragma unroll
        for (int u = 0; u < NG; u++) {
            const int i = min(tid + u * kCtbThreads, n_g - 1);
            const int co = div_small(i, inv_gstr), off = co * OHW + (i - co * gstr);
            gv[u] = gb[off];
            yv[u] = yb[off];
        }
    } else {
        const f32x4* gsrc = reinterpret_cast<const f32x4*>(a.g + (size_t)b0 * a.Cout * OHW);
        const f32x4* ysrc = bwd ? reinterpret_cast<const f32x4*>(a.yout + (size_t)b0 * a.Cout * OHW) : gsrc;
#pragma unroll
        for (int u = 0; u < NG; u++) {
            const int i = min(tid + u * kCtbThreads, n_g - 1);
            gv[u] = gsrc[i];
            yv[u] = ysrc[i];
        }
    }
    const int n_a = BAND ? 16 * astr : nimg * 16 * HW / 4;
    GT av[NA];
    if constexpr (BAND) {
        const float* ab = a.ain + (((size_t)b0 * a.Cin + cb * 16) * a.H + y0) * a.W;
#pragma unroll
        for (int u = 0; u < NA; u++) {
            const int i = min(tid + u * kCtbThreads, n_a - 1);
            const int c = div_small(i, inv_astr);
            av[u] = ab[c * HW + (i - c * astr)];
        }
    } else {
        const int n_a4 = 16 * HW / 4;
        const float inv_na4 = 1.0f / (float)n_a4;
#pragma unroll
        for (int u = 0; u < NA; u++) {
            const int i = min(tid + u * kCtbThreads, n_a - 1);
            const int im = div_small(i, inv_na4), rem = i - im * n_a4;
            av[u] = reinterpret_cast<const f32x4*>(a.ain + ((size_t)(b0 + im) * a.Cin + cb * 16) * HW)[rem];
        }
    }
    const int n_w4 = 16 * N / 4;
    f32x4 wr[kCtbW4];
#pragma unroll
    for (int u = 0; u < kCtbW4; u++)
        wr[u] = reinterpret_cast<const f32x4*>(a.w + (size_t)cb * 16 * N)[min(tid + u * kCtbThreads, n_w4 - 1)];
#pragma unroll
    for (int u = 0; u < NG; u++) asm volatile("" : "+v"(gv[u]), "+v"(yv[u]));
#pragma unroll
    for (int u = 0; u < NA; u++) asm volatile("" : "+v"(av[u]));
#pragma unroll
    for (int u = 0; u < kCtbW4; u++) asm volatile("" : "+v"(wr[u]));

    bn_consts(a.bn_out, cout4, false);
    bn_consts(a.bn_in, cin4, false, 64);
    if (designated && a.bg.stats) {
        for (int c = tid; c < a.bg.C; c += kCtbThreads) {
            double sb = 0.0, sg = 0.0;
            for (int sh = 0; sh < kStatShards; sh++) {
                sb += a.bg.stats[((size_t)sh * a.bg.C + c) * 4 + 2];
                sg += a.bg.stats[((size_t)sh * a.bg.C + c) * 4 + 3];
            }
            a.bg.beta_acc[c] = sb * a.bg.scale;
            a.bg.gamma_acc[c] = sg * a.bg.scale;
        }
    }
    if (tid < 32 * kCtbWaves) lstat[tid] = 0.f;
#pragma unroll
    for (int u = 0; u < NA; u++) {
        const int i = tid + u * kCtbThreads;
        if (i < n_a) reinterpret_cast<GT*>(araw)[i] = av[u];
    }
    {
        const float inv_n = 1.0f / (float)N;
#pragma unroll
        for (int u = 0; u < kCtbW4; u++) {
            const int i = tid + u * kCtbThreads;
            if (i < n_w4) {
                const int row = div_small(4 * i, inv_n);
                float* d = wl + row * a.wstr + (4 * i - row * N);
                d[0] = wr[u][0]; d[1] = wr[u][1]; d[2] = wr[u][2]; d[3] = wr[u][3];
            }
        }
    }
    for (int p = tid; p < P; p += kCtbThreads) {
        const int im = div_small(p, inv_hw), pi = p - im * (nrow * a.W);
        const int y = div_small(pi, inv_w), x = pi - y * a.W;
        pos_g[p] = im * a.Cout * gstr + 2 * y * a.OW + 2 * x;
        pos_a[p] = im * 16 * astr + pi;
        pos_o[p] = im * a.Cin * HW + y0 * a.W + pi;
    }
// ... 185 lines not shown
```

### cae_tools_amd/csrc/kernels_ctlds.h

```cpp
#pragma once
#include "kernels_gemm.h"

namespace cae {

struct CtFwd {
    int B, Cin, H, W, Cout, OH, OW, QH, QW;
    int PW, plane;
    int tiles;
    int rt;
    int ks;
    int tg;
    const float* in;
    BnDesc bn_in;
    const float* w;
    const float* bias;
    float* out;
    double* stats;
};

template <int KH, int KW>
struct CtShape {
    static constexpr int KK = KH * KW;
    static constexpr int KKp = KK | 1;
    static constexpr int WS = 16 * KKp;
};

template <int NP>
__device__ __forceinline__ void ct_load4(const float* __restrict__ ap, const float* __restrict__ bp, int c, int plane, int ws,
                                         float* av, float* bv) {
    constexpr int CSTEP = 4 / NP;
#pragma unroll
    for (int u = 0; u < NP; u++) {
        av[u] = ap[(c + u * CSTEP) * plane];
        bv[u] = bp[(c + u * CSTEP) * ws];
    }
}

constexpr int kCtImgRegs = 12;

template <int KH, int KW>
__global__ void __launch_bounds__(512) k_ct_fwd_lds(CtFwd a) {
    using S = CtShape<KH, KW>;
    constexpr int KK = S::KK, KKp = S::KKp, WS = S::WS;
    constexpr int NJ0 = (KH + 1) / 2, NJ1 = KH / 2, NI0 = (KW + 1) / 2, NI1 = KW / 2;
    constexpr int NP00 = NJ0 * NI0, NP01 = NJ0 * NI1, NP10 = NJ1 * NI0, NP11 = NJ1 * NI1;
    static_assert(KH >= 2 && KH <= 4 && KW >= 2 && KW <= 4, "stride-2 kernels of 2..4 taps per axis");

    kernarg_warm<sizeof(CtFwd)>();
    extern __shared__ double lds_d[];
    double* lstat = lds_d;
    float4* cin4 = reinterpret_cast<float4*>(lstat + 32);
    float* wl = reinterpret_cast<float*>(cin4 + a.Cin);
    float* img = wl + a.Cin * WS;
    float* part = img + ((a.Cin * a.plane + 3) & ~3);
    const int tid = threadIdx.x, nthr = 64 * a.rt * a.ks;
    int b, g;
    if ((a.B & 7) == 0) {
        const int xcd = blockIdx.x & 7, k = blockIdx.x >> 3;
        const int kb = k / a.tg;
        b = xcd + 8 * kb;
        g = k - kb * a.tg;
    } else {
        b = blockIdx.x / a.tg;
        g = blockIdx.x - b * a.tg;
    }
    const int cb = blockIdx.y;

    const int HW = a.H * a.W, n_img = a.Cin * HW;
    const float* src = a.in + (size_t)b * n_img;
    float iv[kCtImgRegs];
#pragma unroll
    for (int u = 0; u < kCtImgRegs; u++) iv[u] = src[min(tid + u * nthr, n_img - 1)];

    const bool bn_designated = blockIdx.x == 0 && blockIdx.y == 0;
    const bool bn_split = a.bn_in.mode == BN_BATCH && a.bn_in.C <= nthr;
    const bool bn_mine = bn_split && tid < a.bn_in.C, bn_upd = bn_designated && a.bn_in.update;
    BnBatchReq bnrq;
    if (bn_mine) bn_batch_request(a.bn_in, tid, bn_upd, bnrq);

    const int ncol = min(16, a.Cout - cb * 16);
    const float* wsrc = a.w + (size_t)cb * 16 * KK;
    const int wstride = a.Cout * KK;
    const bool vec = KKp == KK && ((ncol * KK) & 3) == 0 && (wstride & 3) == 0;
    if (vec) {
        const int n4 = ncol * KK / 4, total4 = a.Cin * n4;
        const float inv_n4 = 1.0f / (float)n4;
        for (int i0 = tid; i0 < total4; i0 += 6 * nthr) {
            f32x4 wv4[6];
            int dst[6];
#pragma unroll
            for (int u = 0; u < 6; u++) {
                const int idx = min(i0 + u * nthr, total4 - 1);
                const int ci = div_small(idx, inv_n4), jq = idx - ci * n4;
                wv4[u] = *reinterpret_cast<const f32x4*>(wsrc + (size_t)ci * wstride + 4 * jq);
                dst[u] = ci * WS + 4 * jq;
            }
            asm volatile("" : "+v"(wv4[0]), "+v"(wv4[1]), "+v"(wv4[2]), "+v"(wv4[3]), "+v"(wv4[4]), "+v"(wv4[5]));
#pragma unroll
            for (int u = 0; u < 6; u++)
// ... 32 lines not shown
    if (tid < 32) lstat[tid] = 0.0;
    {
        const int n4 = (a.Cin * a.plane + 3) >> 2;
        for (int idx = tid; idx < n4; idx += nthr) reinterpret_cast<float4*>(img)[idx] = make_float4(0.f, 0.f, 0.f, 0.f);
    }
    __syncthreads();
    {
        const float inv_hw = 1.0f / (float)HW, inv_w = 1.0f / (float)a.W;
        const bool bn = a.bn_in.mode != BN_NONE;
#pragma unroll
        for (int u = 0; u < kCtImgRegs; u++) {
            const int idx = tid + u * nthr;
            if (idx < n_img) {
                const int ci = div_small(idx, inv_hw), pos = idx - ci * HW;
                const int iy = div_small(pos, inv_w), ix = pos - iy * a.W;
                float v = iv[u];
                if (bn) {
                    const float4 k = cin4[ci];
                    v = fmaxf(0.f, fmaf(v - k.x, k.y, k.z));
                }
                img[ci * a.plane + (iy + 1) * a.PW + ix + 1] = v;
            }
        }
        for (int idx = tid + kCtImgRegs * nthr; idx < n_img; idx += nthr) {
            const int ci = div_small(idx, inv_hw), pos = idx - ci * HW;
            const int iy = div_small(pos, inv_w), ix = pos - iy * a.W;
            float v = src[idx];
            if (bn) {
                const float4 k = cin4[ci];
                v = fmaxf(0.f, fmaf(v - k.x, k.y, k.z));
            }
            img[ci * a.plane + (iy + 1) * a.PW + ix + 1] = v;
        }
    }
    __syncthreads();

    const int wv = tid >> 6, lane = tid & 63;
    const int r = lane & 15, q = lane >> 4;
    const int tl = wv / a.ks, kslot = wv - tl * a.ks;
    const int tile = g * a.rt + tl;
    const bool tile_ok = tile < a.tiles;
    const int Q = a.QH * a.QW;
    const float inv_qw = 1.0f / (float)a.QW;
    const int qi = tile * 16 + r;
    const int qic = (tile_ok && qi < Q) ? qi : 0;
    const int qy = div_small(qic, inv_qw), qx = qic - qy * a.QW;
    const int cper = a.Cin / a.ks, c0 = kslot * cper;
    const int co = cb * 16 + r;
    float bias = a.bias[min(co, a.Cout - 1)];

    f32x4 acc00 = {0.f, 0.f, 0.f, 0.f}, acc01 = acc00, acc10 = acc00, acc11 = acc00;
    if (tile_ok) {
#define CT_PTRS(NP, NI, PY, PX, AP, BP)                                                              \
        const float* AP;                                                                             \
        const float* BP;                                                                             \
        {                                                                                            \
            const int t = q % (NP), dci = q / (NP), j = t / (NI), i = t - j * (NI);                   \
            AP = img + (c0 + dci) * a.plane + (qy - j + 1) * a.PW + (qx - i + 1);                    \
            BP = wl + (c0 + dci) * WS + r * KKp + ((PY) + 2 * j) * KW + (PX) + 2 * i;                \
        }
        CT_PTRS(NP00, NI0, 0, 0, ap00, bp00)
        CT_PTRS(NP01, NI1, 0, 1, ap01, bp01)
        CT_PTRS(NP10, NI0, 1, 0, ap10, bp10)
        CT_PTRS(NP11, NI1, 1, 1, ap11, bp11)
#undef CT_PTRS
        for (int c = 0; c < cper; c += 4) {
            float a00[NP00], b00[NP00], a01[NP01], b01[NP01], a10[NP10], b10[NP10], a11[NP11], b11[NP11];
            ct_load4<NP00>(ap00, bp00, c, a.plane, WS, a00, b00);
            ct_load4<NP01>(ap01, bp01, c, a.plane, WS, a01, b01);
            ct_load4<NP10>(ap10, bp10, c, a.plane, WS, a10, b10);
            ct_load4<NP11>(ap11, bp11, c, a.plane, WS, a11, b11);
#pragma unroll
            for (int u = 0; u < 4; u++) {
                if (u < NP00) acc00 = __builtin_amdgcn_mfma_f32_16x16x4f32(a00[u], b00[u], acc00, 0, 0, 0);
                if (u < NP01) acc01 = __builtin_amdgcn_mfma_f32_16x16x4f32(a01[u], b01[u], acc01, 0, 0, 0);
                if (u < NP10) acc10 = __builtin_amdgcn_mfma_f32_16x16x4f32(a10[u], b10[u], acc10, 0, 0, 0);
                if (u < NP11) acc11 = __builtin_amdgcn_mfma_f32_16x16x4f32(a11[u], b11[u], acc11, 0, 0, 0);
            }
        }
    }
    asm volatile("" : "+v"(bias));

    float s1 = 0.f, s2 = 0.f;
    float* obase = a.out + (size_t)(b * a.Cout + min(co, a.Cout - 1)) * a.OH * a.OW;
    const bool col_ok = tile_ok && co < a.Cout;
    auto emit = [&](int reg, float acc) {
        const int p = reg >> 2, jj = reg & 3;
        const int qo = tile * 16 + q * 4 + jj;
        const int oqy = div_small(min(qo, Q - 1), inv_qw), oqx = min(qo, Q - 1) - oqy * a.QW;
        const int oy = 2 * oqy + (p >> 1), ox = 2 * oqx + (p & 1);
        if (col_ok && qo < Q && oy < a.OH && ox < a.OW) {
            const float v = acc + bias;
            obase[oy * a.OW + ox] = v;
            s1 += v;
            s2 = fmaf(v, v, s2);
        }
    };
    if (a.ks > 1) {
        float* pw = part + wv * 1024 + lane;
#pragma unroll
        for (int jj = 0; jj < 4; jj++) {
            pw[(0 + jj) * 64] = acc00[jj];
            pw[(4 + jj) * 64] = acc01[jj];
            pw[(8 + jj) * 64] = acc10[jj];
            pw[(12 + jj) * 64] = acc11[jj];
        }
        __syncthreads();
        const int rpw = 16 / a.ks;
        const float* pt = part + (tl * a.ks) * 1024 + lane;
        for (int rl = 0; rl < rpw; rl++) {
            const int reg = kslot * rpw + rl;
            float v = 0.f;
            for (int o = 0; o < a.ks; o++) v += pt[o * 1024 + reg * 64];
            emit(reg, v);
        }
    } else {
#pragma unroll
        for (int jj = 0; jj < 4; jj++) {
            emit(0 + jj, acc00[jj]);
            emit(4 + jj, acc01[jj]);
            emit(8 + jj, acc10[jj]);
            emit(12 + jj, acc11[jj]);
        }
    }
    if (a.stats) {
        double d1 = (double)s1, d2 = (double)s2;
        d1 += __shfl_xor(d1, 16, 64); d2 += __shfl_xor(d2, 16, 64);
        d1 += __shfl_xor(d1, 32, 64); d2 += __shfl_xor(d2, 32, 64);
        if (q == 0 && col_ok) {
            atomicAdd(&lstat[2 * r], acc_grid<ACC_STAT>(d1));
            atomicAdd(&lstat[2 * r + 1], acc_grid<ACC_STAT>(d2));
        }
        __syncthreads();
        if (tid < 32) {
            const int c = cb * 16 + (tid >> 1);
            if (c < a.Cout) {
                const int shard = (blockIdx.x + blockIdx.y) & (kStatShards - 1);
                acc_add<ACC_STAT>(&a.stats[((size_t)shard * a.Cout + c) * 4 + (tid & 1)], lstat[tid]);
            }
        }
    }
}

inline size_t ct_fwd_lds_bytes(int Cin, int plane, int KH, int KW, int waves, int ks) {
    const int KKp = (KH * KW) | 1;
    size_t floats = 64 + 4 * (size_t)Cin + (size_t)Cin * 16 * KKp + (((size_t)Cin * plane + 3) & ~(size_t)3);
    if (ks > 1) floats += (size_t)waves * 1024;
    return floats * sizeof(float);
}

}
```

### cae_tools_amd/csrc/kernels_last.h

```cpp
#pragma once
#include <utility>
#include "kernels_s2.h"

namespace cae {

template <class F, int... Is>
__device__ __forceinline__ void static_for_impl(F&& f, std::integer_sequence<int, Is...>) {
    (f(std::integral_constant<int, Is>{}), ...);
}
template <int N, class F>
__device__ __forceinline__ void static_for(F&& f) {
    static_for_impl(f, std::make_integer_sequence<int, N>{});
}

struct S2Last {
    int B, H, W, OH, OW;
    int QH, QW;
    int strips, bands;
    int total;
    const float* in;
    BnDesc bn_in;
    const float* w;
    const float* bias;
    const float* target;
    const int* perm;
    int use_cursor;
    const StepState* st;
    double* losses;
    float inv_count;
    double* bias_acc;
    double* wacc;
    int acc_stride;
    float* gin;
    double* stats_in;
};

constexpr int kLastStripPx = 127;

__device__ __forceinline__ float uniform_f(float v) {
    return __builtin_bit_cast(float, __builtin_amdgcn_readfirstlane(__builtin_bit_cast(int, v)));
}
__device__ __forceinline__ float from_left(float v, float edge) {
    return __builtin_bit_cast(float, __builtin_amdgcn_update_dpp(__builtin_bit_cast(int, edge), __builtin_bit_cast(int, v), 0x138, 0xF, 0xF, false));
}
__device__ __forceinline__ float from_right(float v, float edge) {
    return __builtin_bit_cast(float, __builtin_amdgcn_update_dpp(__builtin_bit_cast(int, edge), __builtin_bit_cast(int, v), 0x130, 0xF, 0xF, false));
}

constexpr int kWsumLd = 68;
constexpr int kWsumScratch = 16 * kWsumLd;
template <int N>
__device__ __forceinline__ void wave_sums_lds(const float (&v)[N], float* scr, float* out, int lane) {
    const int row = lane >> 2, qd = lane & 3;
#pragma unroll
    for (int c0 = 0; c0 < N; c0 += 16) {
#pragma unroll
        for (int i = 0; i < 16; i++)
            if (c0 + i < N) scr[i * kWsumLd + lane] = v[c0 + i];
        const float4* p = reinterpret_cast<const float4*>(scr + row * kWsumLd + 4 * qd);
        const float4 a0 = p[0], a1 = p[4], a2 = p[8], a3 = p[12];
        float t = ((a0.x + a0.y) + (a0.z + a0.w)) + ((a1.x + a1.y) + (a1.z + a1.w)) + ((a2.x + a2.y) + (a2.z + a2.w)) +
                  ((a3.x + a3.y) + (a3.z + a3.w));
        t += dpp_f<0xB1>(t);
        t += dpp_f<0x4E>(t);
        if (qd == 0 && c0 + row < N) out[c0 + row] = t;
    }
}

template <int CIN, int COUT, int KH, int KW, int HB, bool VEC4, bool BN>
__global__ void __launch_bounds__(256) __attribute__((amdgpu_waves_per_eu(1, 2))) k_s2_last_fused(S2Last a) {
    kernarg_warm<sizeof(S2Last)>();
    constexpr int NACC = CIN * COUT * KH * KW;
    constexpr int NRED = NACC + 2 * CIN;
    constexpr int NR = HB + 1;
    static_assert(KH >= 3 && KH <= 4 && KW >= 3 && KW <= 4, "3- or 4-tap stride-2 kernels");
    __shared__ float redf[4 * NRED];
    __shared__ double redd[4 * 2 * COUT];
    __shared__ __attribute__((aligned(16))) float wscr[4 * kWsumScratch];
    __shared__ float xch[4 * CIN * 2 * 64];

    const int tid = threadIdx.x, lane = tid & 63;
    const int wv = __builtin_amdgcn_readfirstlane(tid >> 6);
    const unsigned HW = a.H * a.W, OHW = a.OH * a.OW;

    const int item = blockIdx.x * 4 + wv;
    const bool work = item < a.total;
    const int it = work ? item : 0;
    const int b = it / (a.strips * a.bands);
    const int rem = it - b * (a.strips * a.bands);
    const int band = rem / a.strips, strip = rem - band * a.strips;
    const int m0 = band * HB;
    const bool last_band = band == a.bands - 1, last_strip = strip == a.strips - 1;
    const int n0 = strip * kLastStripPx + 2 * lane;
    const bool multi = a.strips > 1;
    const bool has_below = !multi && work && wv < 3 && band + 1 < a.bands;
    const int nrows = has_below ? HB : NR;
    const bool all_cols = VEC4 && 256 <= a.OW;

    int lane_zero = 0;
    asm volatile("" : "+v"(lane_zero));
    long long bs_v = 0;
    const bool indirect = a.perm != nullptr || a.use_cursor != 0;
    if (indirect) bs_v = (&a.st->batch_start)[lane_zero];
    const int loss_slot_v = (&a.st->loss_slot)[lane_zero];
    double sa = 0.0, sb = 0.0;
    float gam[CIN], bet[CIN], rmn[CIN], rvr[CIN];
    if constexpr (BN) {
        static_assert(CIN <= 8, "one lane per (channel, shard)");
        if (lane < 8 * CIN) {
            const double2 t = *reinterpret_cast<const double2*>(a.bn_in.stats + ((size_t)(lane & 7) * CIN + (lane >> 3)) * 4);
            sa = t.x;
            sb = t.y;
        }
#pragma unroll
        for (int ci = 0; ci < CIN; ci++) {
            gam[ci] = a.bn_in.gamma[ci];
            bet[ci] = a.bn_in.beta[ci];
            rmn[ci] = a.bn_in.rmean[ci];
            rvr[ci] = a.bn_in.rvar[ci];
        }
    }
    float wk[NACC], bk[COUT];
#pragma unroll
    for (int i = 0; i < NACC; i++) wk[i] = a.w[i];
#pragma unroll
    for (int i = 0; i < COUT; i++) bk[i] = a.bias[i];
    asm volatile("" ::: "memory");
    __builtin_amdgcn_sched_barrier(0);
    int perm_val_v;
    if (a.perm) perm_val_v = a.perm[bs_v + b + lane_zero];
    constexpr int NLEFT = VEC4 ? 1 : NR + 1;
    float rin[NR + 1][CIN][2], rleft[NLEFT][CIN];
    float4 tgt[NR][COUT][2];
    {
        const float* inb = a.in + (size_t)b * CIN * HW;
        const int c0 = min(n0, a.W - 1), c1 = min(n0 + 1, a.W - 1), cl = min(max(n0 - 1, 0), a.W - 1);
#pragma unroll
        for (int r = 0; r <= NR; r++) {
            const unsigned ro = (unsigned)min(max(m0 - 1 + r, 0), a.H - 1) * a.W;
#pragma unroll
            for (int ci = 0; ci < CIN; ci++) {
                rin[r][ci][0] = inb[ci * HW + ro + c0];
                rin[r][ci][1] = inb[ci * HW + ro + c1];
                if constexpr (!VEC4) {
                    rleft[r][ci] = 0.f;
                    if (multi && lane == 0) rleft[r][ci] = inb[ci * HW + ro + cl];
                }
            }
        }
        asm volatile("" ::: "memory");
        __builtin_amdgcn_sched_barrier(0);
        const long long bs = ((long long)__builtin_amdgcn_readfirstlane((int)(bs_v >> 32)) << 32) |
                             (unsigned)__builtin_amdgcn_readfirstlane((int)bs_v);
        const long long tb = a.perm ? (long long)__builtin_amdgcn_readfirstlane(perm_val_v) : bs + b;
#pragma unroll
        for (int r = 0; r < NR; r++) {
            if (r >= nrows) break;
#pragma unroll
            for (int co = 0; co < COUT; co++) {
                const float* plane = a.target + ((size_t)tb * COUT + co) * (size_t)OHW;
#pragma unroll
                for (int py = 0; py < 2; py++) {
                    const unsigned ro = (unsigned)min(2 * (m0 + r) + py, a.OH - 1) * a.OW;
                    const int ox = 2 * n0;
                    if constexpr (VEC4) {
                        tgt[r][co][py] = *reinterpret_cast<const float4*>(plane + ro + min(ox, a.OW - 4));
                    } else {
                        tgt[r][co][py].x = plane[ro + min(ox, a.OW - 1)];
                        tgt[r][co][py].y = plane[ro + min(ox + 1, a.OW - 1)];
                        tgt[r][co][py].z = plane[ro + min(ox + 2, a.OW - 1)];
                        tgt[r][co][py].w = plane[ro + min(ox + 3, a.OW - 1)];
                    }
                }
            }
        }
        asm volatile("" ::: "memory");
        __builtin_amdgcn_sched_barrier(0);
    }
#pragma unroll
    for (int i = 0; i < NACC; i++) wk[i] = uniform_f(wk[i]);
#pragma unroll
    for (int i = 0; i < COUT; i++) bk[i] = uniform_f(bk[i]);
    float4 kc[CIN];
#pragma unroll
    for (int ci = 0; ci < CIN; ci++) kc[ci] = make_float4(0.f, 1.f, 0.f, 1.f);
    if constexpr (BN) {
        sa += dpp_d<0xB1>(sa); sb += dpp_d<0xB1>(sb);
        sa += dpp_d<0x4E>(sa); sb += dpp_d<0x4E>(sb);
        sa += dpp_d<0x141>(sa); sb += dpp_d<0x141>(sb);
        const long long ba = __builtin_bit_cast(long long, sa), bb = __builtin_bit_cast(long long, sb);
#pragma unroll
        for (int ci = 0; ci < CIN; ci++) {
            const int lo1 = __builtin_amdgcn_readlane((int)ba, 8 * ci), hi1 = __builtin_amdgcn_readlane((int)(ba >> 32), 8 * ci);
            const int lo2 = __builtin_amdgcn_readlane((int)bb, 8 * ci), hi2 = __builtin_amdgcn_readlane((int)(bb >> 32), 8 * ci);
            const double s1 = __builtin_bit_cast(double, ((long long)hi1 << 32) | (unsigned)lo1);
            const double s2 = __builtin_bit_cast(double, ((long long)hi2 << 32) | (unsigned)lo2);
            const double mu = s1 * a.bn_in.inv_count;
            double var = s2 * a.bn_in.inv_count - mu * mu;
            var = var < 0.0 ? 0.0 : var;
            const float mean = (float)mu;
            const float invstd = 1.0f / sqrtf((float)(var + (double)a.bn_in.eps));
            kc[ci] = make_float4(mean, uniform_f(gam[ci]) * invstd, uniform_f(bet[ci]), invstd);
            if (blockIdx.x == 0 && tid == 0 && a.bn_in.update) {
                a.bn_in.saved[2 * ci] = mean;
                a.bn_in.saved[2 * ci + 1] = invstd;
                a.bn_in.rmean[ci] = (1.f - a.bn_in.momentum) * rmn[ci] + a.bn_in.momentum * mean;
                a.bn_in.rvar[ci] = (1.f - a.bn_in.momentum) * rvr[ci] + a.bn_in.momentum * (float)(var * a.bn_in.unbias);
            }
        }
    }

    float dw[NACC];
#pragma unroll
    for (int i = 0; i < NACC; i++) dw[i] = 0.f;
    float d1[CIN], d2[CIN];
#pragma unroll
    for (int i = 0; i < CIN; i++) d1[i] = d2[i] = 0.f;
    float ls[COUT], gs[COUT];
#pragma unroll
    for (int i = 0; i < COUT; i++) ls[i] = gs[i] = 0.f;

    auto activate = [&](int r, int ci, float (&act)[3]) {
        const int y = m0 - 1 + r;
        const bool rowok = y >= 0 && y < a.H;
        float v0 = rin[r][ci][0], v1 = rin[r][ci][1], vl = VEC4 ? 0.f : rleft[VEC4 ? 0 : r][ci];
        if constexpr (BN) {
// ... 59 lines not shown
#pragma unroll
                for (int py = 0; py < 2; py++) {
                    const float tv[4] = {tgt[r][co][py].x, tgt[r][co][py].y, tgt[r][co][py].z, tgt[r][co][py].w};
                    const bool rowok = 2 * m + py < a.OH;
#pragma unroll
                    for (int q = 0; q < 2; q++)
#pragma unroll
                        for (int px = 0; px < 2; px++) {
                            const int ox = 2 * (n0 + q) + px;
                            const bool valid = rowok && (all_cols || ox < a.OW);
                            const float yh = sigmoid_fast(acc[q][py][px]);
                            const float d = valid ? yh - tv[2 * q + px] : 0.f;
                            const float gv = (2.0f * d * a.inv_count) * (yh * (1.0f - yh));
                            g[co][q][py][px] = gv;
                            if constexpr (VEC4) {
                                if (own_row) { ls[co] = fmaf(d, d, ls[co]); gs[co] += gv; }
                            } else {
                                const bool own = own_row && (q == 0 || lane < 63 || last_strip);
                                const float dl = own ? d : 0.f;
                                ls[co] = fmaf(dl, dl, ls[co]);
                                gs[co] += own ? gv : 0.f;
                            }
                        }
                }
            }
            float P[CIN][2][2][2];
#pragma unroll
            for (int ci = 0; ci < CIN; ci++) {
#pragma unroll
                for (int q = 0; q < 2; q++)
#pragma unroll
                    for (int j = 0; j < 2; j++)
#pragma unroll
                        for (int i = 0; i < 2; i++) P[ci][q][j][i] = 0.f;
#pragma unroll
                for (int co = 0; co < COUT; co++) {
                    const float* wc = &wk[(ci * COUT + co) * KH * KW];
#pragma unroll
                    for (int q = 0; q < 2; q++) {
                        const bool ownq = VEC4 || q == 0 || lane < 63 || last_strip;
#pragma unroll
                        for (int j = 0; j < 2; j++)
#pragma unroll
                            for (int i = 0; i < 2; i++) {
                                const float av = j ? actP[ci][1 + q - i] : actN[ci][1 + q - i];
                                const float avw = ownq ? av : 0.f;
#pragma unroll
                                for (int py = 0; py < 2; py++)
#pragma unroll
                                    for (int px = 0; px < 2; px++)
                                        if (py + 2 * j < KH && px + 2 * i < KW) {
                                            const int t = (py + 2 * j) * KW + px + 2 * i;
                                            P[ci][q][j][i] = fmaf(g[co][q][py][px], wc[t], P[ci][q][j][i]);
                                            if (own_row) dw[(ci * COUT + co) * KH * KW + t] = fmaf(avw, g[co][q][py][px], dw[(ci * COUT + co) * KH * KW + t]);
                                        }
                            }
                    }
                }
            }
            const int y = m - 1;
            const bool emit = r >= 1 && y < a.H;
            float tj1[CIN][2], tj0[CIN][2];
#pragma unroll
            for (int ci = 0; ci < CIN; ci++) {
                tj1[ci][0] = P[ci][0][1][0] + P[ci][1][1][1];
                tj0[ci][0] = P[ci][0][0][0] + P[ci][1][0][1];
                tj1[ci][1] = P[ci][1][1][0] + from_right(P[ci][0][1][1], 0.f);
                tj0[ci][1] = P[ci][1][0][0] + from_right(P[ci][0][0][1], 0.f);
                if (r == 0) { xsave[ci][0] = tj1[ci][0]; xsave[ci][1] = tj1[ci][1]; }
            }
            if (emit) {
                const bool p0 = n0 < a.W, p1 = n0 + 1 < a.W && lane < 63;
#pragma unroll
                for (int ci = 0; ci < CIN; ci++) {
                    float gv0 = carry[ci][0] + tj1[ci][0], gv1 = carry[ci][1] + tj1[ci][1];
                    if constexpr (BN) {
                        const float e0 = rin[r][ci][0] - kc[ci].x, e1 = rin[r][ci][1] - kc[ci].x;
                        gv0 = fmaf(e0, kc[ci].y, kc[ci].z) > 0.f ? gv0 : 0.f;
                        gv1 = fmaf(e1, kc[ci].y, kc[ci].z) > 0.f ? gv1 : 0.f;
                        const float s0 = p0 ? gv0 : 0.f, s1 = p1 ? gv1 : 0.f;
                        d1[ci] += s0 + s1;
                        d2[ci] = fmaf(s0, e0 * kc[ci].w, fmaf(s1, e1 * kc[ci].w, d2[ci]));
                    }
                    float* gp = a.gin + (size_t)(b * CIN + ci) * HW + (unsigned)y * a.W + n0;
                    if (p0) {
                        gp[0] = gv0;
                        gp[p1 ? 1 : 0] = p1 ? gv1 : gv0;
                    }
                }
            }
#pragma unroll
            for (int ci = 0; ci < CIN; ci++) {
                carry[ci][0] = tj0[ci][0];
                carry[ci][1] = tj0[ci][1];
#pragma unroll
                for (int k = 0; k < 3; k++) actP[ci][k] = actN[ci][k];
            }
            }
            if constexpr (r == 0) {
#pragma unroll
                for (int ci = 0; ci < CIN; ci++) {
                    xch[((wv * CIN + ci) * 2 + 0) * 64 + lane] = xsave[ci][0];
                    xch[((wv * CIN + ci) * 2 + 1) * 64 + lane] = xsave[ci][1];
                }
                __syncthreads();
            }
        });
    }
    if (has_below) {
        const int y = m0 + HB - 1;
        if (y < a.H) {
            const bool p0 = n0 < a.W, p1 = n0 + 1 < a.W && lane < 63;
#pragma unroll
            for (int ci = 0; ci < CIN; ci++) {
                float gv0 = carry[ci][0] + xch[(((wv + 1) * CIN + ci) * 2 + 0) * 64 + lane];
                float gv1 = carry[ci][1] + xch[(((wv + 1) * CIN + ci) * 2 + 1) * 64 + lane];
                if constexpr (BN) {
                    const float e0 = rin[HB][ci][0] - kc[ci].x, e1 = rin[HB][ci][1] - kc[ci].x;
                    gv0 = fmaf(e0, kc[ci].y, kc[ci].z) > 0.f ? gv0 : 0.f;
                    gv1 = fmaf(e1, kc[ci].y, kc[ci].z) > 0.f ? gv1 : 0.f;
                    const float s0 = p0 ? gv0 : 0.f, s1 = p1 ? gv1 : 0.f;
                    d1[ci] += s0 + s1;
                    d2[ci] = fmaf(s0, e0 * kc[ci].w, fmaf(s1, e1 * kc[ci].w, d2[ci]));
                }
                float* gp = a.gin + (size_t)(b * CIN + ci) * HW + (unsigned)y * a.W + n0;
                if (p0) {
                    gp[0] = gv0;
                    gp[p1 ? 1 : 0] = p1 ? gv1 : gv0;
                }
            }
        }
    }

    {
        float red[NRED];
#pragma unroll
        for (int i = 0; i < NACC; i++) red[i] = dw[i];
#pragma unroll
        for (int c = 0; c < CIN; c++) {
            red[NACC + 2 * c] = d1[c];
            red[NACC + 2 * c + 1] = d2[c];
        }
        wave_sums_lds<NRED>(red, wscr + wv * kWsumScratch, redf + wv * NRED, lane);
    }
#pragma unroll
    for (int co = 0; co < COUT; co++) {
        const double t1 = wave_sum_lane63((double)ls[co] * (double)a.inv_count), t2 = wave_sum_lane63((double)gs[co]);
        if (lane == 63) {
            redd[(wv * COUT + co) * 2] = t1;
            redd[(wv * COUT + co) * 2 + 1] = t2;
        }
    }
    __syncthreads();
    const int shard = blockIdx.x & (kStatShards - 1);
    for (int j = tid; j < NRED + 2 * COUT; j += 256) {
        if (j < NRED) {
            const double s = (double)redf[j] + (double)redf[NRED + j] + (double)redf[2 * NRED + j] + (double)redf[3 * NRED + j];
            if (j < NACC) {
                acc_add<ACC_GRAD>(&a.wacc[(size_t)shard * a.acc_stride + j], s);
            } else if (a.stats_in) {
                const int jj = j - NACC;
                acc_add<ACC_GRAD>(&a.stats_in[((size_t)shard * CIN + (jj >> 1)) * 4 + 2 + (jj & 1)], s);
            }
        } else {
            const int q = j - NRED, co = q >> 1, which = q & 1;
            double s = 0.0;
#pragma unroll
            for (int w = 0; w < 4; w++) s += redd[(w * COUT + co) * 2 + which];
            if (which == 0) acc_add<ACC_GRAD>(&a.losses[(size_t)loss_slot_v * kStatShards + shard], s);
            else acc_add<ACC_GRAD>(&a.bias_acc[(size_t)shard * a.acc_stride + co], s);
        }
    }
    asm volatile("" :: "v"(perm_val_v));
}

}
```

### cae_tools_amd/csrc/kernels_rows.h

```cpp
#pragma once
#include "kernels_last.h"

namespace cae {

struct S2Rows {
    int B, H, W, OH, OW;
    int QH;
    int bands;
    int groups;
    const float* g;
    const float* yout;
    BnDesc bn_out;
    const float* ain;
    BnDesc bn_in;
    const float* w;
    float* gin;
    double* stats_in;
    double* wacc;
    int wacc_stride;
    BnGradOut bg;
};

template <int CIN, int CT, int COUT, int KH, int KW, int HB, int IMGS, int D>
__global__ void __launch_bounds__(256) __attribute__((amdgpu_waves_per_eu(1, 2))) k_s2_bwd_rows(S2Rows a) {
    kernarg_warm<sizeof(S2Rows)>();
    constexpr int CS = CIN / CT;
    constexpr int NB = 4 / CS;
    constexpr int LW = 64 / IMGS;
    constexpr int NACC = CT * COUT * KH * KW;
    constexpr int NRED = NACC + 2 * CT;
    constexpr int NR = HB + 1;
    static_assert(CS * NB == 4 && CS * CT == CIN, "four waves");
    static_assert(KH == 3 && KW == 3, "3x3 stride-2 kernels");
    static_assert(CIN <= 8 && COUT <= 8, "one lane per (channel, shard) in the BatchNorm prologue");
    __shared__ float redf[4 * NRED];
    __shared__ __attribute__((aligned(16))) float wscr[4 * kWsumScratch];
    __shared__ float xch[NB > 1 ? 4 * CT * 64 : 1];
    __shared__ __attribute__((aligned(16))) float wl[CIN * COUT * 12];

    const int tid = threadIdx.x, lane = tid & 63;
    const int wv = __builtin_amdgcn_readfirstlane(tid >> 6);
    const int cgrp = wv % CS, bsel = wv / CS;
    const int c0 = cgrp * CT;
    const int sub = lane / LW, n = lane - sub * LW;
    const unsigned HW = a.H * a.W, OHW = a.OH * a.OW;

    const int wg_bands = (a.bands + NB - 1) / NB;
    const int grp = blockIdx.x / wg_bands, bg0 = blockIdx.x - grp * wg_bands;
    const int band = bg0 * NB + bsel;
    const bool band_ok = band < a.bands;
    const int m0 = band * HB;
    const int b = grp * IMGS + sub;
    const bool img_ok = b < a.B;
    const int bc = img_ok ? b : a.B - 1;
    const bool has_below = NB > 1 && bsel + 1 < NB && band + 1 < a.bands;
    const int nrows = has_below ? HB : NR;

    float4 ko[COUT], ki[CT];
    double sa = 0.0, sb = 0.0;
    if (lane < 8 * COUT) {
        const double2 t = *reinterpret_cast<const double2*>(a.bn_out.stats + ((size_t)(lane & 7) * COUT + (lane >> 3)) * 4 + 2);
        sa = t.x;
        sb = t.y;
    }
    float mean_o[COUT], istd_o[COUT], gam_o[COUT];
#pragma unroll
    for (int co = 0; co < COUT; co++) {
        mean_o[co] = a.bn_out.saved[2 * co];
        istd_o[co] = a.bn_out.saved[2 * co + 1];
        gam_o[co] = a.bn_out.gamma[co];
    }
    float mean_i[CT], istd_i[CT], gam_i[CT], bet_i[CT];
#pragma unroll
    for (int c = 0; c < CT; c++) {
        mean_i[c] = a.bn_in.saved[2 * (c0 + c)];
        istd_i[c] = a.bn_in.saved[2 * (c0 + c) + 1];
        gam_i[c] = a.bn_in.gamma[c0 + c];
        bet_i[c] = a.bn_in.beta[c0 + c];
    }
    constexpr int NWL = (CIN * COUT * 12 + 255) / 256;
    float wreg[NWL];
#pragma unroll
    for (int u = 0; u < NWL; u++) {
        const int i = min(tid + 256 * u, CIN * COUT * 12 - 1), cc = i / 12, t = i - cc * 12;
        wreg[u] = a.w[cc * 9 + min(t, 8)];
    }
    asm volatile("" ::: "memory");
    __builtin_amdgcn_sched_barrier(0);

    float2 rg[NR][COUT][2], ry[NR][COUT][2];
    float rin[NR + 1][CT];
    const float* gb = a.g + (size_t)bc * COUT * OHW;
    const float* yb = a.yout + (size_t)bc * COUT * OHW;
    const float* ib = a.ain + ((size_t)bc * CIN + c0) * HW;
    const bool pair_ok = 2 * n + 1 < a.OW;
    const int oxc = pair_ok ? 2 * n : min(max(2 * n - 1, 0), a.OW - 2);
    const int xc = min(n, a.W - 1);
    const bool last_band = band == a.bands - 1;
    auto load_in = [&](auto R) {
        constexpr int r = decltype(R)::value;
        const unsigned ro = (unsigned)min(max(m0 - 1 + r, 0), a.H - 1) * a.W;
#pragma unroll
        for (int c = 0; c < CT; c++) rin[r][c] = ib[c * HW + ro + xc];
    };
    auto load_g = [&](auto R) {
        constexpr int r = decltype(R)::value;
        if (r >= nrows) return;
#pragma unroll
        for (int co = 0; co < COUT; co++)
#pragma unroll
            for (int py = 0; py < 2; py++) {
                const unsigned off = co * OHW + (unsigned)min(2 * (m0 + r) + py, a.OH - 1) * a.OW + oxc;
                rg[r][co][py] = *reinterpret_cast<const float2*>(gb + off);
                ry[r][co][py] = *reinterpret_cast<const float2*>(yb + off);
            }
    };
    load_in(std::integral_constant<int, 0>{});
    static_for<(D < NR ? D : NR)>([&](auto R) {
        constexpr int r = decltype(R)::value;
        load_in(std::integral_constant<int, r + 1>{});
        load_g(R);
    });
    __builtin_amdgcn_sched_barrier(0);
    {
        sa += dpp_d<0xB1>(sa); sb += dpp_d<0xB1>(sb);
        sa += dpp_d<0x4E>(sa); sb += dpp_d<0x4E>(sb);
        sa += dpp_d<0x141>(sa); sb += dpp_d<0x141>(sb);
        const long long ba = __builtin_bit_cast(long long, sa), bb = __builtin_bit_cast(long long, sb);
#pragma unroll
        for (int co = 0; co < COUT; co++) {
            const int lo1 = __builtin_amdgcn_readlane((int)ba, 8 * co), hi1 = __builtin_amdgcn_readlane((int)(ba >> 32), 8 * co);
            const int lo2 = __builtin_amdgcn_readlane((int)bb, 8 * co), hi2 = __builtin_amdgcn_readlane((int)(bb >> 32), 8 * co);
            const double dbeta = __builtin_bit_cast(double, ((long long)hi1 << 32) | (unsigned)lo1);
            const double dgamma = __builtin_bit_cast(double, ((long long)hi2 << 32) | (unsigned)lo2);
            const float mean = uniform_f(mean_o[co]), invstd = uniform_f(istd_o[co]);
            const float scale = uniform_f(gam_o[co]) * invstd;
            ko[co] = make_float4(mean, scale, (float)((double)scale * dbeta * a.bn_out.inv_count),
                                 (float)((double)scale * (double)invstd * dgamma * a.bn_out.inv_count));
            if (blockIdx.x == 0 && tid == 0 && a.bg.stats) {
                a.bg.beta_acc[co] = dbeta * a.bg.scale;
                a.bg.gamma_acc[co] = dgamma * a.bg.scale;
            }
        }
#pragma unroll
        for (int c = 0; c < CT; c++) {
            const float invstd = uniform_f(istd_i[c]);
            ki[c] = make_float4(uniform_f(mean_i[c]), uniform_f(gam_i[c]) * invstd, uniform_f(bet_i[c]), invstd);
        }
#pragma unroll
        for (int u = 0; u < NWL; u++) {
            const int i = tid + 256 * u;
            if (i < CIN * COUT * 12) wl[i] = (i % 12) < 9 ? wreg[u] : 0.f;
        }
    }
    __syncthreads();

    float dw[NACC];
#pragma unroll
    for (int i = 0; i < NACC; i++) dw[i] = 0.f;
    float d1[CT], d2[CT];
#pragma unroll
    for (int c = 0; c < CT; c++) d1[c] = d2[c] = 0.f;

    auto activate = [&](int r, int c, float (&act)[2]) {
        const int y = m0 - 1 + r;
        const float v = fmaxf(0.f, fmaf(rin[r][c] - ki[c].x, ki[c].y, ki[c].z));
        act[1] = (y >= 0 && y < a.H && n < a.W) ? v : 0.f;
        const float left = from_left(act[1], 0.f);
        act[0] = n == 0 ? 0.f : left;
    };
    float actP[CT][2], carry[CT];
#pragma unroll
    for (int c = 0; c < CT; c++) {
        activate(0, c, actP[c]);
        carry[c] = 0.f;
    }
    float xsave[CT];
#pragma unroll
    for (int c = 0; c < CT; c++) xsave[c] = 0.f;

    static_for<NR>([&](auto R) {
        constexpr int r = decltype(R)::value;
        const int m = m0 + r;
        if constexpr (r + D < NR) {
            load_in(std::integral_constant<int, r + D + 1>{});
            load_g(std::integral_constant<int, r + D>{});
        }
        if (r < nrows && m < a.QH && band_ok) {
            const bool own_row = r < HB || last_band;
            float actN[CT][2];
#pragma unroll
            for (int c = 0; c < CT; c++) activate(r + 1, c, actN[c]);
            float gy[COUT][2][2];
#pragma unroll
            for (int co = 0; co < COUT; co++)
#pragma unroll
                for (int py = 0; py < 2; py++) {
                    const bool rowok = img_ok && 2 * m + py < a.OH;
                    const float g0 = pair_ok ? rg[r][co][py].x : rg[r][co][py].y, g1 = rg[r][co][py].y;
                    const float y0 = pair_ok ? ry[r][co][py].x : ry[r][co][py].y, y1 = ry[r][co][py].y;
                    const float v0 = ko[co].y * g0 - ko[co].z - (y0 - ko[co].x) * ko[co].w;
                    const float v1 = ko[co].y * g1 - ko[co].z - (y1 - ko[co].x) * ko[co].w;
                    gy[co][py][0] = (rowok && 2 * n < a.OW) ? v0 : 0.f;
                    gy[co][py][1] = (rowok && 2 * n + 1 < a.OW) ? v1 : 0.f;
                }
            int wofs = 0;
            asm volatile("" : "+v"(wofs));
            float P[CT][2][2];
#pragma unroll
            for (int c = 0; c < CT; c++) {
#pragma unroll
                for (int j = 0; j < 2; j++)
#pragma unroll
                    for (int i = 0; i < 2; i++) P[c][j][i] = 0.f;
#pragma unroll
                for (int co = 0; co < COUT; co++) {
                    float wc[12];
                    {
                        const float4* wq = reinterpret_cast<const float4*>(&wl[((c0 + c) * COUT + co) * 12 + wofs]);
                        const float4 w0 = wq[0], w1 = wq[1], w2 = wq[2];
                        wc[0] = w0.x; wc[1] = w0.y; wc[2] = w0.z; wc[3] = w0.w; wc[4] = w1.x; wc[5] = w1.y; wc[6] = w1.z; wc[7] = w1.w;
                        wc[8] = w2.x; wc[9] = w2.y; wc[10] = w2.z; wc[11] = w2.w;
                    }
#pragma unroll
                    for (int j = 0; j < 2; j++)
#pragma unroll
                        for (int i = 0; i < 2; i++) {
                            const float av = j ? actP[c][1 - i] : actN[c][1 - i];
#pragma unroll
                            for (int py = 0; py < 2; py++)
#pragma unroll
                                for (int px = 0; px < 2; px++)
                                    if (py + 2 * j < KH && px + 2 * i < KW) {
                                        const int t = (py + 2 * j) * KW + px + 2 * i;
                                        P[c][j][i] = fmaf(gy[co][py][px], wc[t], P[c][j][i]);
                                        if (own_row) dw[(c * COUT + co) * KH * KW + t] = fmaf(av, gy[co][py][px], dw[(c * COUT + co) * KH * KW + t]);
                                    }
                        }
                }
            }
            const int y = m - 1;
#pragma unroll
            for (int c = 0; c < CT; c++) {
                const float rj1 = from_right(P[c][1][1], 0.f), rj0 = from_right(P[c][0][1], 0.f);
                const float tj1 = P[c][1][0] + (n == LW - 1 ? 0.f : rj1);
                const float tj0 = P[c][0][0] + (n == LW - 1 ? 0.f : rj0);
                if (r == 0) xsave[c] = tj1;
                if (r >= 1 && y < a.H) {
                    float gv = carry[c] + tj1;
                    const float e = rin[r][c] - ki[c].x;
                    gv = fmaf(e, ki[c].y, ki[c].z) > 0.f ? gv : 0.f;
                    const bool pok = img_ok && n < a.W;
                    const float s = pok ? gv : 0.f;
                    d1[c] += s;
                    d2[c] = fmaf(s, e * ki[c].w, d2[c]);
                    if (pok) a.gin[((size_t)b * CIN + c0 + c) * HW + (unsigned)y * a.W + n] = gv;
                }
                carry[c] = tj0;
                actP[c][0] = actN[c][0];
                actP[c][1] = actN[c][1];
            }
        }
        if constexpr (r == 0 && NB > 1) {
#pragma unroll
            for (int c = 0; c < CT; c++) xch[(wv * CT + c) * 64 + lane] = xsave[c];
            __syncthreads();
        }
    });
    if constexpr (NB > 1) {
        if (has_below && band_ok) {
            const int y = m0 + HB - 1;
            if (y < a.H) {
#pragma unroll
                for (int c = 0; c < CT; c++) {
                    float gv = carry[c] + xch[((wv + CS) * CT + c) * 64 + lane];
                    const float e = rin[HB][c] - ki[c].x;
                    gv = fmaf(e, ki[c].y, ki[c].z) > 0.f ? gv : 0.f;
                    const bool pok = img_ok && n < a.W;
                    const float s = pok ? gv : 0.f;
                    d1[c] += s;
                    d2[c] = fmaf(s, e * ki[c].w, d2[c]);
                    if (pok) a.gin[((size_t)b * CIN + c0 + c) * HW + (unsigned)y * a.W + n] = gv;
                }
            }
        }
    }

    {
        float red[NRED];
#pragma unroll
        for (int i = 0; i < NACC; i++) red[i] = dw[i];
#pragma unroll
        for (int c = 0; c < CT; c++) {
            red[NACC + 2 * c] = d1[c];
            red[NACC + 2 * c + 1] = d2[c];
        }
        wave_sums_lds<NRED>(red, wscr + wv * kWsumScratch, redf + wv * NRED, lane);
    }
    __syncthreads();
    const int shard = blockIdx.x & (kStatShards - 1);
    for (int i = tid; i < CS * NRED; i += 256) {
        const int gsel = i / NRED, j = i - gsel * NRED;
        double s = 0.0;
#pragma unroll
        for (int q = 0; q < NB; q++) s += (double)redf[(q * CS + gsel) * NRED + j];
        if (j < NACC) {
            acc_add<ACC_GRAD>(&a.wacc[(size_t)shard * a.wacc_stride + (size_t)gsel * NACC + j], s);
        } else {
            const int jj = j - NACC;
            acc_add<ACC_GRAD>(&a.stats_in[((size_t)shard * CIN + gsel * CT + (jj >> 1)) * 4 + 2 + (jj & 1)], s);
        }
    }
}

}

namespace cae {

struct S2FwdRows {
    int B, H, W, OH, OW;
    int QH;
    int bands, groups;
    const float* in;
    BnDesc bn_in;
    const float* w;
    const float* bias;
    float* out;
    double* stats;
};

template <int CIN, int COUT, int HB, int IMGS>
__global__ void __launch_bounds__(256) k_s2_fwd_rows(S2FwdRows a) {
    kernarg_warm<sizeof(S2FwdRows)>();
    constexpr int KH = 3, KW = 3;
    constexpr int LW = 64 / IMGS;
    constexpr int NRED = 2 * COUT;
    static_assert(CIN <= 8, "one lane per (channel, shard) in the BatchNorm prologue");
    __shared__ float redf[4 * NRED];
    __shared__ __attribute__((aligned(16))) float wscr[4 * kWsumScratch];
    __shared__ __attribute__((aligned(16))) float wl[CIN * COUT * 12];

    const int tid = threadIdx.x, lane = tid & 63;
    const int wv = __builtin_amdgcn_readfirstlane(tid >> 6);
    const int sub = lane / LW, n = lane - sub * LW;
    const unsigned HW = a.H * a.W, OHW = a.OH * a.OW;
    const int wg_bands = (a.bands + 3) / 4;
    const int grp = blockIdx.x / wg_bands, bg0 = blockIdx.x - grp * wg_bands;
    const int band = bg0 * 4 + wv;
    const bool band_ok = band < a.bands;
    const int m0 = band * HB;
    const int b = grp * IMGS + sub;
    const bool img_ok = b < a.B;
    const int bc = img_ok ? b : a.B - 1;

    float4 ki[CIN];
    const bool batch = a.bn_in.mode == BN_BATCH;
    double sa = 0.0, sb = 0.0;
    if (batch && lane < 8 * CIN) {
        const double2 t = *reinterpret_cast<const double2*>(a.bn_in.stats + ((size_t)(lane & 7) * CIN + (lane >> 3)) * 4);
        sa = t.x;
        sb = t.y;
    }
    float gam[CIN], bet[CIN], rmn[CIN], rvr[CIN];
#pragma unroll
    for (int c = 0; c < CIN; c++) {
        gam[c] = a.bn_in.gamma[c];
        bet[c] = a.bn_in.beta[c];
        rmn[c] = a.bn_in.rmean[c];
        rvr[c] = a.bn_in.rvar[c];
    }
    constexpr int NWL = (CIN * COUT * 12 + 255) / 256;
    float wreg[NWL];
#pragma unroll
    for (int u = 0; u < NWL; u++) {
        const int i = min(tid + 256 * u, CIN * COUT * 12 - 1), cc = i / 12, t = i - cc * 12;
        wreg[u] = a.w[cc * 9 + min(t, 8)];
    }
    float bk[COUT];
#pragma unroll
    for (int co = 0; co < COUT; co++) bk[co] = a.bias[co];
    asm volatile("" ::: "memory");
    __builtin_amdgcn_sched_barrier(0);

    float rin[HB + 1][CIN];
    {
        const float* ib = a.in + (size_t)bc * CIN * HW;
        const int xc = min(n, a.W - 1);
#pragma unroll
        for (int r = 0; r <= HB; r++) {
            const unsigned ro = (unsigned)min(max(m0 - 1 + r, 0), a.H - 1) * a.W;
#pragma unroll
            for (int c = 0; c < CIN; c++) rin[r][c] = ib[c * HW + ro + xc];
        }
    }
    __builtin_amdgcn_sched_barrier(0);
    {
        sa += dpp_d<0xB1>(sa); sb += dpp_d<0xB1>(sb);
        sa += dpp_d<0x4E>(sa); sb += dpp_d<0x4E>(sb);
        sa += dpp_d<0x141>(sa); sb += dpp_d<0x141>(sb);
        const long long ba = __builtin_bit_cast(long long, sa), bb = __builtin_bit_cast(long long, sb);
#pragma unroll
        for (int c = 0; c < CIN; c++) {
            float mean, invstd;
            if (batch) {
                const int lo1 = __builtin_amdgcn_readlane((int)ba, 8 * c), hi1 = __builtin_amdgcn_readlane((int)(ba >> 32), 8 * c);
                const int lo2 = __builtin_amdgcn_readlane((int)bb, 8 * c), hi2 = __builtin_amdgcn_readlane((int)(bb >> 32), 8 * c);
                const double s1 = __builtin_bit_cast(double, ((long long)hi1 << 32) | (unsigned)lo1);
                const double s2 = __builtin_bit_cast(double, ((long long)hi2 << 32) | (unsigned)lo2);
                const double mu = s1 * a.bn_in.inv_count;
                double var = s2 * a.bn_in.inv_count - mu * mu;
                var = var < 0.0 ? 0.0 : var;
                mean = (float)mu;
                invstd = 1.0f / sqrtf((float)(var + (double)a.bn_in.eps));
                if (blockIdx.x == 0 && tid == 0 && a.bn_in.update) {
                    a.bn_in.saved[2 * c] = mean;
                    a.bn_in.saved[2 * c + 1] = invstd;
                    a.bn_in.rmean[c] = (1.f - a.bn_in.momentum) * rmn[c] + a.bn_in.momentum * mean;
                    a.bn_in.rvar[c] = (1.f - a.bn_in.momentum) * rvr[c] + a.bn_in.momentum * (float)(var * a.bn_in.unbias);
                }
            } else {
                mean = uniform_f(rmn[c]);
                invstd = 1.0f / sqrtf(uniform_f(rvr[c]) + a.bn_in.eps);
            }
            ki[c] = make_float4(mean, uniform_f(gam[c]) * invstd, uniform_f(bet[c]), invstd);
        }
#pragma unroll
        for (int u = 0; u < NWL; u++) {
            const int i = tid + 256 * u;
            if (i < CIN * COUT * 12) wl[i] = (i % 12) < 9 ? wreg[u] : 0.f;
        }
#pragma unroll
        for (int co = 0; co < COUT; co++) bk[co] = uniform_f(bk[co]);
    }
    __syncthreads();

    auto activate = [&](int r, int c, float (&act)[2]) {
        const int y = m0 - 1 + r;
        const float v = fmaxf(0.f, fmaf(rin[r][c] - ki[c].x, ki[c].y, ki[c].z));
        act[1] = (y >= 0 && y < a.H && n < a.W) ? v : 0.f;
        const float left = from_left(act[1], 0.f);
        act[0] = n == 0 ? 0.f : left;
    };
    float actP[CIN][2];
#pragma unroll
    for (int c = 0; c < CIN; c++) activate(0, c, actP[c]);
    float s1[COUT], s2[COUT];
#pragma unroll
    for (int co = 0; co < COUT; co++) s1[co] = s2[co] = 0.f;
    const bool pair_ok = 2 * n + 1 < a.OW;
    float* ob = a.out + (size_t)bc * COUT * OHW;

    static_for<HB>([&](auto R) {
        constexpr int r = decltype(R)::value;
        const int m = m0 + r;
        if (m < a.QH && band_ok) {
            float actN[CIN][2];
#pragma unroll
            for (int c = 0; c < CIN; c++) activate(r + 1, c, actN[c]);
            int wofs = 0;
            asm volatile("" : "+v"(wofs));
#pragma unroll
            for (int co = 0; co < COUT; co++) {
                float acc[2][2] = {{bk[co], bk[co]}, {bk[co], bk[co]}};
#pragma unroll
                for (int c = 0; c < CIN; c++) {
                    float wc[12];
                    {
                        const float4* wq = reinterpret_cast<const float4*>(&wl[(c * COUT + co) * 12 + wofs]);
                        const float4 w0 = wq[0], w1 = wq[1], w2 = wq[2];
                        wc[0] = w0.x; wc[1] = w0.y; wc[2] = w0.z; wc[3] = w0.w; wc[4] = w1.x; wc[5] = w1.y; wc[6] = w1.z; wc[7] = w1.w;
                        wc[8] = w2.x; wc[9] = w2.y; wc[10] = w2.z; wc[11] = w2.w;
                    }
#pragma unroll
                    for (int j = 0; j < 2; j++)
#pragma unroll
                        for (int i = 0; i < 2; i++) {
                            const float av = j ? actP[c][1 - i] : actN[c][1 - i];
#pragma unroll
                            for (int py = 0; py < 2; py++)
#pragma unroll
                                for (int px = 0; px < 2; px++)
                                    if (py + 2 * j < KH && px + 2 * i < KW)
                                        acc[py][px] = fmaf(av, wc[(py + 2 * j) * KW + px + 2 * i], acc[py][px]);
                        }
                }
#pragma unroll
                for (int py = 0; py < 2; py++) {
                    const int oy = 2 * m + py;
                    const bool ok0 = img_ok && oy < a.OH && 2 * n < a.OW, ok1 = ok0 && pair_ok;
                    float* op = ob + co * OHW + (unsigned)min(oy, a.OH - 1) * a.OW + min(2 * n, a.OW - 1);
                    if (ok1) *reinterpret_cast<float2*>(op) = make_float2(acc[py][0], acc[py][1]);
                    else if (ok0) op[0] = acc[py][0];
                    const float v0 = ok0 ? acc[py][0] : 0.f, v1 = ok1 ? acc[py][1] : 0.f;
                    s1[co] += v0 + v1;
                    s2[co] = fmaf(v0, v0, fmaf(v1, v1, s2[co]));
                }
            }
#pragma unroll
            for (int c = 0; c < CIN; c++) {
                actP[c][0] = actN[c][0];
                actP[c][1] = actN[c][1];
            }
        }
    });
    if (!a.stats) return;
    {
        float red[NRED];
#pragma unroll
        for (int co = 0; co < COUT; co++) {
            red[2 * co] = s1[co];
            red[2 * co + 1] = s2[co];
        }
        wave_sums_lds<NRED>(red, wscr + wv * kWsumScratch, redf + wv * NRED, lane);
    }
    __syncthreads();
    if (tid < NRED) {
        const double s = (double)redf[tid] + (double)redf[NRED + tid] + (double)redf[2 * NRED + tid] + (double)redf[3 * NRED + tid];
        acc_add<ACC_STAT>(&a.stats[((size_t)(blockIdx.x & (kStatShards - 1)) * COUT + (tid >> 1)) * 4 + (tid & 1)], s);
    }
}

}
```

### cae_tools_amd/engine.py

```python
import ctypes as C
from collections import OrderedDict

import numpy as np
import torch

from . import _lib
from ._engine_base import TEST, TRAIN, SpecPlan, _spec_layers, _to_c, require_gpu
from ._lib import CaeError, check


class EnginePlan(SpecPlan):

    PREFIX = "cae_"

    def bn_prefixes(self):
        return [n[: -len(".running_mean")] for n in self.tensors if n.endswith(".running_mean")]

    def set_kernel_mode(self, mode):
        check(self.lib.cae_set_kernel_mode(self.handle, int(mode)))

    def kernel_plan(self, batch, train):
        buf = C.create_string_buffer(1 << 16)
        check(self.lib.cae_debug_plan(self.handle, int(batch), 1 if train else 0, buf, len(buf)))
        plan = {}
        for line in buf.value.decode().splitlines():
            (name, *fields) = line.split()
            plan[name] = dict(f.split("=", 1) for f in fields)
        return plan


class HipEngine(EnginePlan):

    def __init__(self, spec, fc_size, latent_size, max_batch, device=None, graph=True, specialised=True):
        require_gpu()
        super().__init__(spec, fc_size, latent_size, max_batch)
        self._bind(device, grads=True, buffers=True)
        check(self.lib.cae_set_graph_mode(self.handle, 1 if graph else 0))
        check(self.lib.cae_set_kernel_mode(self.handle, int(specialised) if isinstance(specialised, int) and not isinstance(specialised, bool) else (1 if specialised else 0)))
        torch.cuda.synchronize(self.device)
        self.num_batches_tracked = 0
        self.adam_steps = 0
        self._datasets = {}
        self._keep = []
        self.loss_slots = int(self.lib.cae_loss_slots(self.handle))
        self._slot = 0
        self._cursor = None

    def grad_view(self, name):
        (arena, off, numel, shape) = self.tensors[name]
        assert arena == 0
        return self.grads[off:off + numel].view(shape)

    def export_state(self):
        (enc, dec) = super().export_state()
        return self._ordered(enc), self._ordered(dec)

    @staticmethod
    def _ordered(sd):
        order = {"weight": 0, "bias": 1, "running_mean": 2, "running_var": 3, "num_batches_tracked": 4}
        groups = OrderedDict()
        for k in sd:
            groups.setdefault(k.rsplit(".", 1)[0], []).append(k)
        out = OrderedDict()
        for g, keys in groups.items():
            for k in sorted(keys, key=lambda s: order[s.rsplit(".", 1)[1]]):
                out[k] = sd[k]
        return out

    def reset_optimizer(self):
        self.sync()
        self.exp_avg.zero_()
        self.exp_avg_sq.zero_()
        self.adam_steps = 0
        torch.cuda.synchronize(self.device)
        check(self.lib.cae_set_adam_step(self.handle, 0))

    def load_optimizer_state(self, moments, step):
        self.sync()
        for name, (m, v) in moments.items():
            (arena, off, numel, shape) = self.tensors[name]
            self.exp_avg[off:off + numel].copy_(torch.as_tensor(m, dtype=torch.float32).reshape(-1).to(self.device))
            self.exp_avg_sq[off:off + numel].copy_(torch.as_tensor(v, dtype=torch.float32).reshape(-1).to(self.device))
        torch.cuda.synchronize(self.device)
        self.adam_steps = int(step)
        check(self.lib.cae_set_adam_step(self.handle, int(step)))

    def set_hyper(self, lr=1e-3, betas=(0.9, 0.999), eps=1e-8, weight_decay=1e-5):
        check(self.lib.cae_set_hyper(self.handle, float(lr), float(betas[0]), float(betas[1]), float(eps),
                                     float(weight_decay)))

    def set_lr(self, lr):
        check(self.lib.cae_set_lr(self.handle, float(lr)))

    def _same_device(self, a, what):
        if a.device != self.device:
            raise CaeError(f"{what} lives on {a.device} but this engine runs on {self.device} "
                           "(select the rank's GPU before creating data sets: cae_tools_amd.dp.select_device)")

    def set_dataset(self, which, x, t=None):
        for name, a, shp in (("x", x, self.in_shape), ("t", t, self.out_shape)):
            if a is None:
                continue
            if a.dtype != torch.float32 or not a.is_cuda or not a.is_contiguous():
                raise CaeError(f"dataset {name} must be a contiguous fp32 CUDA tensor")
            self._same_device(a, f"dataset {name}")
            if tuple(a.shape[1:]) != tuple(shp):
# ... 429 lines not shown
```

Measured before the change: 382,200.

## Pad decoder activation maps to 32-float row pitch between row kernels

Decoder BN activation and gradient buffers get a row pitch rounded up to a multiple of 32 floats for widths of 31 or more. Producer and consumer kernels (rows fwd/bwd, ct_lds fwd, ct_bwd band path, fused last) take separate input and output pitches, but only when every kernel touching a map supports pitch. The aim is aligned rows for coalesced and vector loads and stores, together with float2 loads and stores in the last-layer kernel. It costs more workspace memory, a planner that must pick the same pitch for every producer and consumer, and a strided host copy for debug readback.

Measured after the change: 379,200. Within noise of the previous version (-0.8%).

```diff
diff --git a/cae_tools_amd/csrc/engine.hip b/cae_tools_amd/csrc/engine.hip
--- a/cae_tools_amd/csrc/engine.hip
+++ b/cae_tools_amd/csrc/engine.hip
@@ -65,7 +65,9 @@
     int64_t rm_off, rv_off;
     int64_t act_off, grad_off;
     int sh_w = -1, sh_b = -1;
+    int pitch = 0;
     int64_t out_elems() const { return (int64_t)cout * hout * wout; }
+    int64_t out_pitched() const { return (int64_t)cout * hout * pitch; }
     int64_t in_elems() const { return (int64_t)cin * hin * win; }
 };
 
@@ -110,6 +112,9 @@
     bool variational = false;
     int64_t off_vz = 0, off_vgz = 0, off_zlast = 0;
     cae_internal::TrunkHooks hooks{nullptr, nullptr, nullptr};
+    bool dense_maps = false;
+    int last_batch = 0;
+    bool last_train = false, last_ext = false;
     bool gather_fwd = false;
     int ctbwd_mask = 0;
     int ctbwd_auto = 0;
@@ -618,12 +623,12 @@
 }
 
 void ct_fwd_launch(cae_engine* e, const StepArgs& a, const ConvLayer& L, int layer, const float* in, const BnDesc& bn_in,
-                   float* out, double* stats) {
+                   float* out, int out_pitch, double* stats) {
     CtFwd c;
     int waves = 0;
     size_t lds = 0;
     (void)ct_fwd_plan(e, a.batch, L, layer, c, waves, lds);
-    c.in = in; c.bn_in = bn_in; c.w = e->params + L.w_off; c.bias = e->params + L.b_off; c.out = out; c.stats = stats;
+    c.in = in; c.bn_in = bn_in; c.w = e->params + L.w_off; c.bias = e->params + L.b_off; c.out = out; c.OP = out_pitch; c.stats = stats;
     dim3 grid((unsigned)(a.batch * c.tg), (unsigned)((L.cout + 15) / 16));
     ProfScope _p(e, a.train ? "ct_convt_fwd" : "ct_convt_eval", layer, f4((double)a.batch * (L.in_elems() + L.out_elems())));
     if (L.kh == 3 && L.kw == 3) ct_fwd_go<3, 3>(c, grid, 64 * waves, lds, e->stream);
@@ -886,6 +891,45 @@
     return DB_GENERIC;
 }
 
+struct CtBwdSplit { int parts, bands, hb; };
+
+CtBwdSplit ct_bwd_split(const ConvLayer& L, const CtBwdPlan& cp) {
+    CtBwdSplit r{std::max(1, std::min(8, 256 / (cp.groups * (L.cin / 16)))), 0, 0};
+    if (cp.imgs == 1 && r.parts > 1) {
+        const int hb = (L.hin + r.parts - 1) / r.parts, bands = (L.hin + hb - 1) / hb;
+        const int gstr = (2 * hb + 1) * L.wout, astr = hb * L.win;
+        if (bands > 1 && L.cout * gstr <= 8 * kCtbThreads && 16 * astr <= 2 * kCtbThreads) {
+            r.bands = bands;
+            r.hb = hb;
+            r.parts = bands;
+        }
+    }
+    return r;
+}
+
+int rule_pitch(int w) { return w >= 31 ? (w + 31) / 32 * 32 : w; }
+
+int map_pitch(const cae_engine* e, int l, int B, bool train, bool external_loss) {
+    const int n = (int)e->dec.size();
+    const ConvLayer& L = e->dec[l];
+    if (l + 1 >= n || L.pitch == L.wout || e->dense_maps || e->variational) return L.wout;
+    const DecFwdK pf = choose_dec_fwd(e, L, l, B, train, external_loss);
+    const DecFwdK cf = choose_dec_fwd(e, e->dec[l + 1], l + 1, B, train, external_loss);
+    if ((pf != DF_ROWS && pf != DF_CT_LDS) || (cf != DF_ROWS && cf != DF_FUSED_LAST)) return L.wout;
+    if (train) {
+        const DecBwdK ob = choose_dec_bwd(e, L, l, B, external_loss);
+        const DecBwdK ib = choose_dec_bwd(e, e->dec[l + 1], l + 1, B, external_loss);
+        if (ib != DB_ROWS && ib != DB_FUSED_LAST) return L.wout;
+        if (ob == DB_CT_LDS) {
+            CtBwdPlan cp;
+            if (!ct_bwd_plan(e, B, L, l, cp) || ct_bwd_split(L, cp).bands == 0) return L.wout;
+        } else if (ob != DB_ROWS) {
+            return L.wout;
+        }
+    }
+    return L.pitch;
+}
+
 StepTail narrow_tail(cae_engine* e, bool with_step_tail, int batch_inc) {
     StepTail t = step_tail_of(e, batch_inc, 1);
     if (!with_step_tail) {
@@ -1094,6 +1138,8 @@
             S2FwdRows f;
             memset(&f, 0, sizeof f);
             f.B = B; f.H = L.hin; f.W = L.win; f.OH = L.hout; f.OW = L.wout;
+            f.IP = map_pitch(e, (int)l - 1, B, a.train, a.external_loss);
+            f.OP = map_pitch(e, (int)l, B, a.train, a.external_loss);
             f.in = small.p; f.bn_in = bns;
             f.w = e->params + L.w_off; f.bias = e->params + L.b_off;
             f.out = ep.out;
@@ -1140,7 +1186,8 @@
             continue;
         }
         if (fk == DF_CT_LDS) {
-            ct_fwd_launch(e, a, L, (int)l, small.p, bns, ep.out, a.train ? ep.stats : nullptr);
+            ct_fwd_launch(e, a, L, (int)l, small.p, bns, ep.out, last ? L.wout : map_pitch(e, (int)l, B, a.train, a.external_loss),
+                          a.train ? ep.stats : nullptr);
             if (a.train)
                 if (int rc = sync_bn_table(e, a, L.bn_index)) return rc;
             continue;
@@ -1211,6 +1258,7 @@
             S2Last f;
             memset(&f, 0, sizeof f);
             f.B = B; f.H = L.hin; f.W = L.win; f.OH = L.hout; f.OW = L.wout;
+            f.IP = l > 0 ? map_pitch(e, l - 1, B, true, a.external_loss) : L.win;
             f.in = ain.p;
             f.w = e->params + L.w_off;
             f.bias = e->params + L.b_off;
@@ -1244,6 +1292,8 @@
             S2Rows f;
             memset(&f, 0, sizeof f);
             f.B = B; f.H = L.hin; f.W = L.win; f.OH = L.hout; f.OW = L.wout;
+            f.IP = map_pitch(e, l - 1, B, true, a.external_loss);
+            f.OP = map_pitch(e, l, B, true, a.external_loss);
             f.g = gy.p; f.yout = gy.q; f.bn_out = bng;
             f.ain = ain.p; f.bn_in = bna;
             f.w = e->params + L.w_off;
@@ -1305,6 +1355,7 @@
             memset(&c, 0, sizeof c);
             c.B = B; c.Cin = L.cin; c.H = L.hin; c.W = L.win; c.Cout = L.cout; c.OH = L.hout; c.OW = L.wout;
             c.imgs = imgs; c.wstr = wstr;
+            c.GP = last ? L.wout : map_pitch(e, l, B, true, a.external_loss);
             c.g = gy.p; c.yout = gy.q; c.bn_out = bng;
             c.ain = ain.p; c.bn_in = bna;
             c.w = e->params + L.w_off;
@@ -1330,18 +1381,15 @@
             }
             ProfScope _p(e, "ct_convt_bwd", l,
                          f4((double)B * (L.out_elems() * (last ? 1.0 : 2.0) + L.in_elems() * (l == 0 ? 1.0 : 2.0))));
-            int parts = std::max(1, std::min(8, 256 / (groups * (L.cin / 16))));
+            const CtBwdSplit sp = ct_bwd_split(L, cp);
+            const int parts = sp.parts;
             size_t lds_launch = lds;
-            if (imgs == 1 && parts > 1) {
-                const int hb = (L.hin + parts - 1) / parts, bands = (L.hin + hb - 1) / hb;
-                const int gstr = (2 * hb + 1) * L.wout, astr = hb * L.win;
-                if (bands > 1 && L.cout * gstr <= 8 * kCtbThreads && 16 * astr <= 2 * kCtbThreads) {
-                    c.bands = bands;
-                    c.hb = hb;
-                    parts = bands;
-                    lds_launch = (32 * (size_t)kCtbWaves + 4 * (size_t)(L.cin + L.cout) + (size_t)L.cout * gstr + 4 + 16 * (size_t)astr + 4 +
-                                  16 * (size_t)wstr + 3 * (size_t)astr + (size_t)kCtbWaves * 16 * 17 + 8) * sizeof(float);
-                }
+            if (sp.bands) {
+                const int gstr = (2 * sp.hb + 1) * L.wout, astr = sp.hb * L.win;
+                c.bands = sp.bands;
+                c.hb = sp.hb;
+                lds_launch = (32 * (size_t)kCtbWaves + 4 * (size_t)(L.cin + L.cout) + (size_t)L.cout * gstr + 4 + 16 * (size_t)astr + 4 +
+                              16 * (size_t)wstr + 3 * (size_t)astr + (size_t)kCtbWaves * 16 * 17 + 8) * sizeof(float);
             }
             if (cae_internal::ctbwd_launch(&c, sizeof c, (unsigned)groups, (unsigned)(L.cin / 16), (unsigned)parts, lds_launch, s))
                 return fail(CAE_ERR_ARG, "k_ct_bwd_lds: argument layout mismatch");
@@ -1730,6 +1778,11 @@
 
 int run_op(cae_engine* e, int op, const StepArgs& a, bool cacheable) {
     if (int rc = push_lr(e)) return rc;
+    if (op != OP_ADAM && a.part != 1) {
+        e->last_batch = a.batch;
+        e->last_train = a.train;
+        e->last_ext = a.external_loss;
+    }
     if (!e->graph_mode || !cacheable || e->stream == nullptr || e->profiling)
         return e->capture_only ? CAE_OK : launch_op(e, op, a);
     auto key = std::make_tuple(op, a.which, a.batch, a.global_batch, (const void*)a.perm, a.nsteps, a.cursor_inc,
@@ -1953,9 +2006,10 @@
         e->fc[i].grad_off = carve(mb * e->fc[i].nout * 4);
     }
     for (auto& L : e->dec) {
+        L.pitch = L.has_bn ? rule_pitch(L.wout) : L.wout;
         if (!L.has_bn) continue;
-        L.act_off = carve(mb * L.out_elems() * 4);
-        L.grad_off = carve(mb * L.out_elems() * 4);
+        L.act_off = carve(mb * L.out_pitched() * 4);
+        L.grad_off = carve(mb * L.out_pitched() * 4);
     }
     e->off_glast = carve(mb * e->dec.back().out_elems() * 4);
     e->off_xbatch = carve((mb * e->enc[0].in_elems() + e->enc[0].cout) * 4);
@@ -2038,7 +2092,10 @@
     if (!e) return fail(CAE_ERR_ARG, "null engine");
     const int ctb = (specialised & 2) ? 0x7fffffff : e->ctbwd_auto;
     const bool gather = (specialised & 4) != 0;
-    if (e->use_s2 != ((specialised & 1) != 0) || ctb != e->ctbwd_mask || gather != e->gather_fwd) e->drop_graphs();
+    const bool dense = (specialised & 8) != 0;
+    if (e->use_s2 != ((specialised & 1) != 0) || ctb != e->ctbwd_mask || gather != e->gather_fwd || dense != e->dense_maps)
+        e->drop_graphs();
+    e->dense_maps = dense;
     e->use_s2 = (specialised & 1) != 0;
     e->ctbwd_mask = ctb;
     e->gather_fwd = gather;
@@ -2444,6 +2501,17 @@
         if (!L) return fail(CAE_ERR_ARG, "layer index out of range");
         src = e->ws + (w == "act" ? L->act_off : L->grad_off);
         n = mb * L->out_elems();
+        const int dl = index - n_enc;
+        const int pitch = dl >= 0 ? map_pitch(e, dl, std::max(e->last_batch, 1), e->last_train, e->last_ext) : L->wout;
+        if (pitch != L->wout) {
+            if (n > cap) n = cap;
+            const int64_t rows = std::min<int64_t>((int64_t)e->last_batch * L->cout * L->hout, n / L->wout);
+            memset(host_out, 0, (size_t)n * 4);
+            HIP_TRY(hipStreamSynchronize(e->stream));
+            HIP_TRY(hipMemcpy2D(host_out, (size_t)L->wout * 4, src, (size_t)pitch * 4, (size_t)L->wout * 4, (size_t)rows,
+                                hipMemcpyDeviceToHost));
+            return n;
+        }
     } else if (w == "glast") {
         src = e->ws + e->off_glast;
         n = mb * e->dec.back().out_elems();
@@ -2540,7 +2608,7 @@
 int cae_debug_plan(const cae_engine* e, int batch, int train, char* out, int64_t out_bytes) {
     if (!e || !out || out_bytes < 1) return fail(CAE_ERR_ARG, "cae_debug_plan: bad argument");
     if (batch < 1 || batch > e->max_batch) return fail(CAE_ERR_ARG, "cae_debug_plan: batch %d outside 1 .. %d", batch, e->max_batch);
-    const bool tr = train != 0, ext = e->variational;
+    const bool tr = (train & 1) != 0, ext = e->variational;
     const StepArgs a{0, nullptr, batch, batch, batch, tr, true, nullptr, nullptr, false};
     std::string s;
     char line[256];
@@ -2607,6 +2675,14 @@
         size_t lds = 0;
         snprintf(line, sizeof line, "tail bwd=%s\n", !tr ? "-" : (tail_plan(e, a, t, lds) ? "fused" : "layers"));
         s += line;
+    }
+    if (train & 2) {
+        s += "maps";
+        for (int l = 0; l + 1 < (int)e->dec.size(); l++) {
+            snprintf(line, sizeof line, " dec%d=%d", l, map_pitch(e, l, batch, tr, ext));
+            s += line;
+        }
+        s += "\n";
     }
     if ((int64_t)s.size() + 1 > out_bytes)
         return fail(CAE_ERR_ARG, "cae_debug_plan: the report needs %zu bytes, got %lld", s.size() + 1, (long long)out_bytes);
diff --git a/cae_tools_amd/csrc/kernels_ctbwd.h b/cae_tools_amd/csrc/kernels_ctbwd.h
--- a/cae_tools_amd/csrc/kernels_ctbwd.h
+++ b/cae_tools_amd/csrc/kernels_ctbwd.h
@@ -8,6 +8,7 @@
     int imgs;
     int bands, hb;
     int wstr;
+    int GP;
     const float* g;
     const float* yout;
     BnDesc bn_out;
@@ -74,12 +75,14 @@
     const int n_g = BAND ? a.Cout * gstr : nimg * a.Cout * OHW / 4;
     GT gv[NG], yv[NG];
     if constexpr (BAND) {
-        const float* gb = a.g + ((size_t)b0 * a.Cout * a.OH + 2 * y0) * a.OW;
-        const float* yb = bwd ? a.yout + ((size_t)b0 * a.Cout * a.OH + 2 * y0) * a.OW : gb;
+        const float* gb = a.g + ((size_t)b0 * a.Cout * a.OH + 2 * y0) * a.GP;
+        const float* yb = bwd ? a.yout + ((size_t)b0 * a.Cout * a.OH + 2 * y0) * a.GP : gb;
+        const float inv_ow = 1.0f / (float)a.OW;
 #pragma unroll
         for (int u = 0; u < NG; u++) {
             const int i = min(tid + u * kCtbThreads, n_g - 1);
-            const int co = div_small(i, inv_gstr), off = co * OHW + (i - co * gstr);
+            const int co = div_small(i, inv_gstr), rem = i - co * gstr, row = div_small(rem, inv_ow);
+            const int off = (co * a.OH + row) * a.GP + (rem - row * a.OW);
             gv[u] = gb[off];
             yv[u] = yb[off];
         }
diff --git a/cae_tools_amd/csrc/kernels_ctlds.h b/cae_tools_amd/csrc/kernels_ctlds.h
--- a/cae_tools_amd/csrc/kernels_ctlds.h
+++ b/cae_tools_amd/csrc/kernels_ctlds.h
@@ -15,6 +15,7 @@
     const float* w;
     const float* bias;
     float* out;
+    int OP;
     double* stats;
 };
 
@@ -213,7 +214,7 @@
     asm volatile("" : "+v"(bias));
 
     float s1 = 0.f, s2 = 0.f;
-    float* obase = a.out + (size_t)(b * a.Cout + min(co, a.Cout - 1)) * a.OH * a.OW;
+    float* obase = a.out + (size_t)(b * a.Cout + min(co, a.Cout - 1)) * a.OH * a.OP;
     const bool col_ok = tile_ok && co < a.Cout;
     auto emit = [&](int reg, float acc) {
         const int p = reg >> 2, jj = reg & 3;
@@ -222,7 +223,7 @@
         const int oy = 2 * oqy + (p >> 1), ox = 2 * oqx + (p & 1);
         if (col_ok && qo < Q && oy < a.OH && ox < a.OW) {
             const float v = acc + bias;
-            obase[oy * a.OW + ox] = v;
+            obase[oy * a.OP + ox] = v;
             s1 += v;
             s2 = fmaf(v, v, s2);
         }
diff --git a/cae_tools_amd/csrc/kernels_last.h b/cae_tools_amd/csrc/kernels_last.h
--- a/cae_tools_amd/csrc/kernels_last.h
+++ b/cae_tools_amd/csrc/kernels_last.h
@@ -15,6 +15,7 @@
 
 struct S2Last {
     int B, H, W, OH, OW;
+    int IP;
     int QH, QW;
     int strips, bands;
     int total;
@@ -81,7 +82,7 @@
 
     const int tid = threadIdx.x, lane = tid & 63;
     const int wv = __builtin_amdgcn_readfirstlane(tid >> 6);
-    const unsigned HW = a.H * a.W, OHW = a.OH * a.OW;
+    const unsigned HW = a.H * a.IP, OHW = a.OH * a.OW;
 
     const int item = blockIdx.x * 4 + wv;
     const bool work = item < a.total;
@@ -135,13 +136,22 @@
     {
         const float* inb = a.in + (size_t)b * CIN * HW;
         const int c0 = min(n0, a.W - 1), c1 = min(n0 + 1, a.W - 1), cl = min(max(n0 - 1, 0), a.W - 1);
+        const bool pair = a.W >= 2;
+        const int cb = min(n0, a.W - 2);
+        const bool second = n0 > cb;
 #pragma unroll
         for (int r = 0; r <= NR; r++) {
-            const unsigned ro = (unsigned)min(max(m0 - 1 + r, 0), a.H - 1) * a.W;
+            const unsigned ro = (unsigned)min(max(m0 - 1 + r, 0), a.H - 1) * a.IP;
 #pragma unroll
             for (int ci = 0; ci < CIN; ci++) {
-                rin[r][ci][0] = inb[ci * HW + ro + c0];
-                rin[r][ci][1] = inb[ci * HW + ro + c1];
+                if (pair) {
+                    const float2 v = *reinterpret_cast<const float2*>(inb + ci * HW + ro + cb);
+                    rin[r][ci][0] = second ? v.y : v.x;
+                    rin[r][ci][1] = v.y;
+                } else {
+                    rin[r][ci][0] = inb[ci * HW + ro + c0];
+                    rin[r][ci][1] = inb[ci * HW + ro + c1];
+                }
                 if constexpr (!VEC4) {
                     rleft[r][ci] = 0.f;
                     if (multi && lane == 0) rleft[r][ci] = inb[ci * HW + ro + cl];
@@ -367,11 +377,9 @@
                         d1[ci] += s0 + s1;
                         d2[ci] = fmaf(s0, e0 * kc[ci].w, fmaf(s1, e1 * kc[ci].w, d2[ci]));
                     }
-                    float* gp = a.gin + (size_t)(b * CIN + ci) * HW + (unsigned)y * a.W + n0;
-                    if (p0) {
-                        gp[0] = gv0;
-                        gp[p1 ? 1 : 0] = p1 ? gv1 : gv0;
-                    }
+                    float* gp = a.gin + (size_t)(b * CIN + ci) * HW + (unsigned)y * a.IP + n0;
+                    if (p1) *reinterpret_cast<float2*>(gp) = make_float2(gv0, gv1);
+                    else if (p0) gp[0] = gv0;
                 }
             }
 #pragma unroll
@@ -408,11 +416,9 @@
                     d1[ci] += s0 + s1;
                     d2[ci] = fmaf(s0, e0 * kc[ci].w, fmaf(s1, e1 * kc[ci].w, d2[ci]));
                 }
-                float* gp = a.gin + (size_t)(b * CIN + ci) * HW + (unsigned)y * a.W + n0;
-                if (p0) {
-                    gp[0] = gv0;
-                    gp[p1 ? 1 : 0] = p1 ? gv1 : gv0;
-                }
+                float* gp = a.gin + (size_t)(b * CIN + ci) * HW + (unsigned)y * a.IP + n0;
+                if (p1) *reinterpret_cast<float2*>(gp) = make_float2(gv0, gv1);
+                else if (p0) gp[0] = gv0;
             }
         }
     }
diff --git a/cae_tools_amd/csrc/kernels_rows.h b/cae_tools_amd/csrc/kernels_rows.h
--- a/cae_tools_amd/csrc/kernels_rows.h
+++ b/cae_tools_amd/csrc/kernels_rows.h
@@ -5,6 +5,7 @@
 
 struct S2Rows {
     int B, H, W, OH, OW;
+    int IP, OP;
     int QH;
     int bands;
     int groups;
@@ -43,7 +44,7 @@
     const int cgrp = wv % CS, bsel = wv / CS;
     const int c0 = cgrp * CT;
     const int sub = lane / LW, n = lane - sub * LW;
-    const unsigned HW = a.H * a.W, OHW = a.OH * a.OW;
+    const unsigned HW = a.H * a.IP, OHW = a.OH * a.OP;
 
     const int wg_bands = (a.bands + NB - 1) / NB;
     const int grp = blockIdx.x / wg_bands, bg0 = blockIdx.x - grp * wg_bands;
@@ -99,7 +100,7 @@
     const bool last_band = band == a.bands - 1;
     auto load_in = [&](auto R) {
         constexpr int r = decltype(R)::value;
-        const unsigned ro = (unsigned)min(max(m0 - 1 + r, 0), a.H - 1) * a.W;
+        const unsigned ro = (unsigned)min(max(m0 - 1 + r, 0), a.H - 1) * a.IP;
 #pragma unroll
         for (int c = 0; c < CT; c++) rin[r][c] = ib[c * HW + ro + xc];
     };
@@ -110,7 +111,7 @@
         for (int co = 0; co < COUT; co++)
 #pragma unroll
             for (int py = 0; py < 2; py++) {
-                const unsigned off = co * OHW + (unsigned)min(2 * (m0 + r) + py, a.OH - 1) * a.OW + oxc;
+                const unsigned off = co * OHW + (unsigned)min(2 * (m0 + r) + py, a.OH - 1) * a.OP + oxc;
                 rg[r][co][py] = *reinterpret_cast<const float2*>(gb + off);
                 ry[r][co][py] = *reinterpret_cast<const float2*>(yb + off);
             }
@@ -254,7 +255,7 @@
                     const float s = pok ? gv : 0.f;
                     d1[c] += s;
                     d2[c] = fmaf(s, e * ki[c].w, d2[c]);
-                    if (pok) a.gin[((size_t)b * CIN + c0 + c) * HW + (unsigned)y * a.W + n] = gv;
+                    if (pok) a.gin[((size_t)b * CIN + c0 + c) * HW + (unsigned)y * a.IP + n] = gv;
                 }
                 carry[c] = tj0;
                 actP[c][0] = actN[c][0];
@@ -280,7 +281,7 @@
                     const float s = pok ? gv : 0.f;
                     d1[c] += s;
                     d2[c] = fmaf(s, e * ki[c].w, d2[c]);
-                    if (pok) a.gin[((size_t)b * CIN + c0 + c) * HW + (unsigned)y * a.W + n] = gv;
+                    if (pok) a.gin[((size_t)b * CIN + c0 + c) * HW + (unsigned)y * a.IP + n] = gv;
                 }
             }
         }
@@ -319,6 +320,7 @@
 
 struct S2FwdRows {
     int B, H, W, OH, OW;
+    int IP, OP;
     int QH;
     int bands, groups;
     const float* in;
@@ -343,7 +345,7 @@
     const int tid = threadIdx.x, lane = tid & 63;
     const int wv = __builtin_amdgcn_readfirstlane(tid >> 6);
     const int sub = lane / LW, n = lane - sub * LW;
-    const unsigned HW = a.H * a.W, OHW = a.OH * a.OW;
+    const unsigned HW = a.H * a.IP, OHW = a.OH * a.OP;
     const int wg_bands = (a.bands + 3) / 4;
     const int grp = blockIdx.x / wg_bands, bg0 = blockIdx.x - grp * wg_bands;
     const int band = bg0 * 4 + wv;
@@ -388,7 +390,7 @@
         const int xc = min(n, a.W - 1);
 #pragma unroll
         for (int r = 0; r <= HB; r++) {
-            const unsigned ro = (unsigned)min(max(m0 - 1 + r, 0), a.H - 1) * a.W;
+            const unsigned ro = (unsigned)min(max(m0 - 1 + r, 0), a.H - 1) * a.IP;
 #pragma unroll
             for (int c = 0; c < CIN; c++) rin[r][c] = ib[c * HW + ro + xc];
         }
@@ -488,7 +490,7 @@
                 for (int py = 0; py < 2; py++) {
                     const int oy = 2 * m + py;
                     const bool ok0 = img_ok && oy < a.OH && 2 * n < a.OW, ok1 = ok0 && pair_ok;
-                    float* op = ob + co * OHW + (unsigned)min(oy, a.OH - 1) * a.OW + min(2 * n, a.OW - 1);
+                    float* op = ob + co * OHW + (unsigned)min(oy, a.OH - 1) * a.OP + min(2 * n, a.OW - 1);
                     if (ok1) *reinterpret_cast<float2*>(op) = make_float2(acc[py][0], acc[py][1]);
                     else if (ok0) op[0] = acc[py][0];
                     const float v0 = ok0 ? acc[py][0] : 0.f, v1 = ok1 ? acc[py][1] : 0.f;
diff --git a/cae_tools_amd/engine.py b/cae_tools_amd/engine.py
--- a/cae_tools_amd/engine.py
+++ b/cae_tools_amd/engine.py
@@ -19,9 +19,9 @@
     def set_kernel_mode(self, mode):
         check(self.lib.cae_set_kernel_mode(self.handle, int(mode)))
 
-    def kernel_plan(self, batch, train):
+    def kernel_plan(self, batch, train, maps=False):
         buf = C.create_string_buffer(1 << 16)
-        check(self.lib.cae_debug_plan(self.handle, int(batch), 1 if train else 0, buf, len(buf)))
+        check(self.lib.cae_debug_plan(self.handle, int(batch), (1 if train else 0) | (2 if maps else 0), buf, len(buf)))
         plan = {}
         for line in buf.value.decode().splitlines():
             (name, *fields) = line.split()
```
